# skywind3000/QuickNet

Hardware: AMD Instinct MI355X
Metric: RS(k,m) FEC encode+decode GiB/s (device-resident) at 1/2/4/8 MI355X (higher is better)
Workload: dtype u8

## Files before the change

### quicknet_amd/csrc/gf256.cpp

```cpp
#include <string.h>

#include <algorithm>
#include <mutex>
#include <vector>

#include "qfec_internal.hpp"

namespace qfec {

namespace {

uint8_t clmul_reduce(uint8_t a, uint8_t b) {
    unsigned acc = 0, x = a;
    for (int i = 0; i < 8; ++i)
        if (b & (1u << i)) acc ^= x << i;
    for (int bit = 14; bit >= 8; --bit)
        if (acc & (1u << bit)) acc ^= 0x11Du << (bit - 8);
    return (uint8_t)acc;
}

Field g_field;
std::once_flag g_field_once;

void build_field() {
    Field& f = g_field;
    for (int a = 0; a < 256; ++a)
        for (int b = 0; b < 256; ++b) f.mul[a][b] = clmul_reduce((uint8_t)a, (uint8_t)b);
    uint8_t x = 1;
    memset(f.log, 0, sizeof(f.log));
    for (int i = 0; i < 255; ++i) {
        f.exp[i] = x;
        f.exp[i + 255] = x;
        f.log[x] = (uint8_t)i;
        x = f.mul[x][2];
    }
    f.exp[510] = f.exp[511] = 0;
    f.log[0] = 255;
    f.inv[0] = 0;
    for (int a = 1; a < 256; ++a) f.inv[a] = f.exp[(255 - f.log[a]) % 255];
}

}

Tuning& tuning() {
    static Tuning t;
    return t;
}

const Field& field() {
    std::call_once(g_field_once, build_field);
    return g_field;
}

DivMagic make_div_magic(uint32_t d) {
    DivMagic m{};
    if (d == 0) d = 1;
    if ((d & (d - 1)) == 0) {
        m.pow2 = 1;
        m.shift = 0;
        while ((1u << m.shift) < d) ++m.shift;
        m.mul = 1;
        return m;
    }
    uint32_t l = 0;
    while ((1ull << l) < d) ++l;
    m.pow2 = 0;
    m.shift = l;
    m.mul = (uint64_t)(((unsigned __int128)1 << (32 + l)) / d) + 1;
    return m;
}

bool gf_invert(uint8_t* a, int k) {
    const Field& f = field();
    std::vector<uint8_t> aug((size_t)k * 2 * k, 0);
    const int w = 2 * k;
    for (int r = 0; r < k; ++r) {
        memcpy(&aug[(size_t)r * w], a + (size_t)r * k, (size_t)k);
        aug[(size_t)r * w + k + r] = 1;
    }
    for (int c = 0; c < k; ++c) {
        int p = c;
        while (p < k && aug[(size_t)p * w + c] == 0) ++p;
        if (p == k) return false;
        if (p != c)
            for (int j = 0; j < w; ++j) std::swap(aug[(size_t)p * w + j], aug[(size_t)c * w + j]);
        uint8_t* pr = &aug[(size_t)c * w];
        const uint8_t s = f.inv[pr[c]];
        for (int j = 0; j < w; ++j) pr[j] = f.mul[s][pr[j]];
        for (int r = 0; r < k; ++r) {
            if (r == c) continue;
            uint8_t* rr = &aug[(size_t)r * w];
            const uint8_t q = rr[c];
            if (!q) continue;
            const uint8_t* mq = f.mul[q];
            for (int j = 0; j < w; ++j) rr[j] ^= mq[pr[j]];
        }
    }
    for (int r = 0; r < k; ++r) memcpy(a + (size_t)r * k, &aug[(size_t)r * w + k], (size_t)k);
    return true;
}

bool gf_invert_rs(uint8_t* a, int k) {
    const Field& f = field();
    std::vector<uint8_t> used((size_t)k, 0);
    std::vector<int> sw_row((size_t)k, -1), sw_col((size_t)k, -1);
    auto row = [&](int r) { return a + (size_t)r * k; };
    for (int s = 0; s < k; ++s) {
        int pr = -1, pc = -1;
        if (!used[s] && row(s)[s]) {
            pr = pc = s;
        } else {
            for (int r = 0; r < k && pc < 0; ++r) {
                if (used[r]) continue;
                for (int c = 0; c < k; ++c)
                    if (!used[c] && row(r)[c]) { pr = r; pc = c; break; }
            }
            if (pc < 0) return false;
        }
        used[pc] = 1;
        if (pr != pc) std::swap_ranges(row(pr), row(pr) + k, row(pc));
        sw_row[s] = pr;
        sw_col[s] = pc;
        uint8_t* p = row(pc);
        if (p[pc] != 1) {
            const uint8_t* sc = f.mul[f.inv[p[pc]]];
            p[pc] = 1;
            for (int c = 0; c < k; ++c) p[c] = sc[p[c]];
        }
        bool unit = true;
        for (int c = 0; c < k && unit; ++c) unit = p[c] == (c == pc);
        if (unit) continue;
        for (int r = 0; r < k; ++r) {
            if (r == pc) continue;
            uint8_t* q = row(r);
            const uint8_t x = q[pc];
            q[pc] = 0;
            if (!x) continue;
            const uint8_t* mx = f.mul[x];
            for (int c = 0; c < k; ++c) q[c] ^= mx[p[c]];
        }
    }
    for (int s = k - 1; s >= 0; --s)
        if (sw_row[s] != sw_col[s])
            for (int r = 0; r < k; ++r) std::swap(row(r)[sw_row[s]], row(r)[sw_col[s]]);
    return true;
}

bool cauchy_rows(int k, int m, std::vector<uint8_t>& out) {
    if (k <= 0 || m <= 0 || k + m > 255) return false;
    const Field& f = field();
    out.assign((size_t)m * k, 0);
    for (int j = 0; j < m; ++j)
        for (int i = 0; i < k; ++i) out[(size_t)j * k + i] = f.inv[(m + i) ^ j];
    return true;
}

bool vandermonde_rows(int k, int m, std::vector<uint8_t>& out) {
    const int n = k + m;
    if (k <= 0 || m < 0 || k > 256 || n > 256) return false;
    const Field& f = field();
    std::vector<uint8_t> v((size_t)n * k, 0);
    v[0] = 1;
    for (int r = 1; r < n; ++r)
        for (int c = 0; c < k; ++c) v[(size_t)r * k + c] = f.exp[((r - 1) * c) % 255];
    std::vector<uint8_t> top(v.begin(), v.begin() + (size_t)k * k);
    if (!gf_invert(top.data(), k)) return false;
    out.assign((size_t)m * k, 0);
    for (int r = 0; r < m; ++r)
        for (int c = 0; c < k; ++c) {
            uint8_t acc = 0;
            const uint8_t* row = &v[(size_t)(k + r) * k];
            for (int i = 0; i < k; ++i) acc ^= f.mul[row[i]][top[(size_t)i * k + c]];
            out[(size_t)r * k + c] = acc;
        }
    return true;
}

static inline uint32_t pack4(uint8_t a, uint8_t b, uint8_t c, uint8_t d) {
    return (uint32_t)a | ((uint32_t)b << 8) | ((uint32_t)c << 16) | ((uint32_t)d << 24);
}

void perm_entry(uint8_t c, uint32_t* o) {
    const Field& f = field();
    const uint8_t* mc = f.mul[c];
    o[0] = pack4(mc[0], mc[1], mc[2], mc[3]);
    o[1] = pack4(mc[4], mc[5], mc[6], mc[7]);
    o[2] = pack4(mc[0], mc[8], mc[16], mc[24]);
    o[3] = pack4(mc[32], mc[40], mc[48], mc[56]);
    o[4] = pack4(mc[0], mc[64], mc[128], mc[192]);
    o[5] = 0;
    o[6] = c ? f.log[c] : 0xFFu;
    o[7] = c;
}

int decode_rows(const uint8_t* P, int k, int m, const uint8_t* marks, std::vector<uint8_t>& rows,
                std::vector<int>& survivors, std::vector<int>& lost, const uint8_t* full) {
    lost.clear();
    survivors.clear();
    for (int i = 0; i < k; ++i) {
        if (marks[i]) lost.push_back(i);
        else survivors.push_back(i);
    }
    const int e = (int)lost.size();
    if (e == 0) return 0;
    for (int j = 0; j < m && (int)survivors.size() < k; ++j)
        if (!marks[k + j]) survivors.push_back(k + j);
    if ((int)survivors.size() < k) return -1;
    std::vector<uint8_t> d((size_t)k * k, 0);
    if (full) {
        for (int r = 0; r < k; ++r) memcpy(&d[(size_t)r * k], full + (size_t)survivors[r] * k, (size_t)k);
        (void)gf_invert_rs(d.data(), k);
    } else {
        for (int r = 0; r < k; ++r) {
            const int s = survivors[r];
            if (s < k) d[(size_t)r * k + s] = 1;
            else memcpy(&d[(size_t)r * k], P + (size_t)(s - k) * k, (size_t)k);
        }
        if (!gf_invert(d.data(), k)) return -1;
    }
    rows.assign((size_t)e * k, 0);
    for (int j = 0; j < e; ++j) memcpy(&rows[(size_t)j * k], &d[(size_t)lost[j] * k], (size_t)k);
    return e;
}

int repair_rows(const uint8_t* P, int k, int m, const uint8_t* marks, std::vector<uint8_t>& rows,
                std::vector<int>& survivors, std::vector<int>& lost, const uint8_t* full, int* e_out) {
    const int n = k + m;
    int t = 0;
    for (int i = 0; i < n; ++i) t += marks[i] ? 1 : 0;
    rows.clear();
    survivors.clear();
    lost.clear();
    if (e_out) *e_out = 0;
    if (t == 0) return 0;
    if (t > m) return -1;
    std::vector<uint8_t> drows;
    std::vector<int> dlost;
    const int e = decode_rows(P, k, m, marks, drows, survivors, dlost, full);
    if (e < 0) return -1;
    if (e_out) *e_out = e;
    lost = dlost;
    for (int j = 0; j < m; ++j)
        if (marks[k + j]) lost.push_back(k + j);
    rows.assign((size_t)t * k, 0);
    if (e) memcpy(rows.data(), drows.data(), (size_t)e * k);
    const Field& f = field();
    std::vector<int> pos((size_t)k, -1);
    for (int c = 0; c < k; ++c)
        if (survivors[c] < k) pos[survivors[c]] = c;
    for (int r = e; r < t; ++r) {
        const uint8_t* pr = P + (size_t)(lost[r] - k) * k;
        uint8_t* out = &rows[(size_t)r * k];
        for (int i = 0; i < k; ++i)
            if (pos[i] >= 0) out[pos[i]] ^= pr[i];
        for (int j = 0; j < e; ++j) {
            const uint8_t q = pr[dlost[j]];
            if (!q) continue;
            const uint8_t* mq = f.mul[q];
            for (int c = 0; c < k; ++c) out[c] ^= mq[drows[(size_t)j * k + c]];
        }
    }
    return t;
}

void build_repair_record(const RecordLayout& L, int k, int t, int e, const uint8_t* rows, const int* survivors,
                         const int* lost, bool rs_quirk, uint32_t* out) {
    memset(out, 0, (size_t)L.hdr * sizeof(uint32_t));
    out[0] = (uint32_t)t;
    out[2] = (uint32_t)e;
    for (int c = 0; c < k; ++c) out[L.surv_off + c] = (uint32_t)survivors[c];
    for (int j = 0; j < t; ++j) out[L.lost_off + j] = (uint32_t)lost[j];
    for (int j = 0; j < t; ++j)
        for (int c = 0; c < k; ++c) out[L.coff + j * k + c] = (uint32_t)rows[(size_t)j * k + c] * (QFEC_TAB_STRIDE * 4);
    if (rs_quirk)
        for (int j = 0; j < e && j < 32; ++j)
            if (rows[(size_t)j * k] == 0) out[1] |= 1u << j;
}

RecordLayout record_layout(int k, int m) {
    RecordLayout L;
    L.surv_off = 4;
    L.lost_off = 4 + k;
    L.coff = (4 + k + m + 7) & ~7;
    L.hdr = (L.coff + m * k + 7) & ~7;
    return L;
}

void build_record(const RecordLayout& L, int k, int e, const uint8_t* rows, const int* survivors,
                  const int* lost, bool rs_quirk, uint32_t* out) {
    memset(out, 0, L.words(e, k) * sizeof(uint32_t));
    out[0] = (uint32_t)e;
    for (int c = 0; c < k; ++c) out[L.surv_off + c] = (uint32_t)survivors[c];
    for (int j = 0; j < e; ++j) out[L.lost_off + j] = (uint32_t)lost[j];
    for (int j = 0; j < e; ++j)
        for (int c = 0; c < k; ++c) {
            uint32_t* t = out + L.hdr + ((size_t)j * k + c) * QFEC_TAB_STRIDE;
            perm_entry(rows[(size_t)j * k + c], t);
            out[L.coff + j * k + c] = (uint32_t)rows[(size_t)j * k + c] * (QFEC_TAB_STRIDE * 4);
        }
    if (rs_quirk)
        for (int j = 0; j < e; ++j)
            if (rows[(size_t)j * k] == 0) {
                out[L.hdr + ((size_t)j * k) * QFEC_TAB_STRIDE + 5] = 1;
                if (j < 32) out[1] |= 1u << j;
            }
}

}
```

### quicknet_amd/csrc/qfec_internal.hpp

```cpp
#pragma once

#include <hip/hip_runtime.h>
#include <stdint.h>

#include <atomic>
#include <vector>

namespace qfec {

constexpr int QFEC_TAB_STRIDE = 8;

constexpr int QFEC_REC_NONE = -1;
constexpr int QFEC_REC_FAIL = -2;
constexpr int QFEC_LE_UNCHECKED = -1;
constexpr int QFEC_LE_LOST = -2;
constexpr int QFEC_LUT_MAX_N = 24;

constexpr int QFEC_VARIANT_PERM_I = 0;
constexpr int QFEC_VARIANT_LDSLOG_I = 1;

struct DivMagic {
    uint64_t mul;
    uint32_t shift;
    uint32_t pow2;
};

DivMagic make_div_magic(uint32_t d);

struct EncodeArgs {
    const uint8_t* data;
    uint8_t* parity;
    const uint32_t* tab;
    const uint8_t* gf_exp;
    const uint8_t* gf_log;
    uint64_t work;
    uint64_t pitch;
    uint64_t dgs, pgs;
    DivMagic cols_div;
    uint32_t cols;
    int k, m;
    int vec16;
    int impl;
    int lds;
    int block;
};

struct ReconArgs {
    uint8_t* data;
    const uint8_t* parity;
    const uint8_t* marks;
    const int32_t* lut;
    const int32_t* group_rec;
    const uint32_t* records;
    unsigned int* failed;
    uint64_t groups;
    uint64_t pitch;
    uint64_t dgs, pgs;
    uint32_t cols;
    int k, m;
    int surv_off, lost_off, hdr;
    int coff;
    const uint32_t* t256;
    int vec16;
    int impl;
    uint32_t wpg;
    uint32_t cols8, wpg8;
    uint32_t cols12, wpg12;
    int rlds;
};

struct RepairArgs {
    uint8_t* data;
    uint8_t* parity;
    const uint8_t* dmarks;
    const uint8_t* pmarks;
    const int32_t* lut;
    const uint32_t* records;
    const uint32_t* t256;
    unsigned int* failed;
    uint64_t groups;
    uint64_t pitch;
    uint64_t dgs, pgs;
    uint32_t cols;
    uint32_t cols8, wpg8;
    int k, m;
    int surv_off, lost_off, coff;
    int vec16;
};

struct VerifyArgs {
    const uint8_t* data;
    const uint8_t* parity;
    const uint32_t* tab;
    unsigned int* bad_rows;
    unsigned int* bad_groups;
    uint64_t work;
    uint64_t pitch;
    uint64_t dgs, pgs;
    DivMagic cols_div;
    uint32_t cols;
    uint32_t block;
    int k, m;
    int vec16;
};

struct LocateArgs {
    const uint8_t* data;
    const uint8_t* parity;
    const uint32_t* tab;
    const uint32_t* rtab;
    unsigned int* bad_rows;
    unsigned int* cand;
    uint64_t work;
    uint64_t pitch;
    uint64_t dgs, pgs;
    DivMagic cols_div;
    uint32_t cols;
    uint32_t block;
    int k, m;
    int vec16;
};

struct LocateFinishArgs {
    const unsigned int* bad_rows;
    const unsigned int* cand;
    int* culprit;
    uint8_t* marks;
    unsigned int* counts;
    uint64_t groups;
    int k, m;
};

struct LocErasedArgs {
    const uint8_t* data;
    const uint8_t* parity;
    const uint8_t* dmarks;
    const uint8_t* pmarks;
    const int32_t* lut;
    const uint32_t* records;
    const uint32_t* t256;
    unsigned int* bad;
    unsigned int* cand;
    uint64_t groups;
    uint64_t pitch;
    uint64_t dgs, pgs;
    uint32_t cols;
    uint32_t cols8, wpg8;
    uint32_t block;
    int k, m;
    int ids_off, aoff, roff;
    int vec16;
};

struct LocErasedFinishArgs {
    const uint8_t* marks;
    const int32_t* lut;
    const uint32_t* records;
    const unsigned int* bad;
    const unsigned int* cand;
    int* culprit;
    uint8_t* marks_out;
    unsigned int* counts;
    uint64_t groups;
    int k, m;
    int ids_off;
    int scrub;
};

struct WireArgs {
    const uint8_t* payload;
    const int64_t* offsets;
    const int32_t* sizes;
    const uint32_t* seq;
    uint8_t* shards;
    uint64_t group_stride;
    uint64_t pitch;
    uint8_t* wire;
    uint64_t wire_pitch;
    int32_t* wire_len;
    uint8_t* marks;
    int32_t* rx_size;
    int32_t* status;
    int32_t* psize;
    uint64_t groups;
    int k, m;
    int checksum;
    int dec_pkt_size;
    int store_nt;
};

hipError_t launch_build_shards(const WireArgs& a, hipStream_t s);
hipError_t launch_pack_fused(const WireArgs& a, const uint32_t* tab, uint32_t* part, hipStream_t s, bool* launched);
struct FrameArgs {
    const uint8_t* in;
    const int32_t* in_len;
    uint8_t* out;
    int32_t* out_len;
    const uint8_t* mask;
    uint32_t* conv_hid;
    int32_t* status;
    uint8_t* info;
    uint64_t rows, in_pitch, out_pitch;
    uint32_t gmask, cmd, protocol;
    int session;
};
hipError_t launch_frame_udp(const FrameArgs& a, hipStream_t s);
struct FrameSend {
    const uint8_t* mask;
    const uint32_t* conv_hid;
    uint32_t gmask, cmd, protocol;
};
struct FrameRecv {
    uint32_t gmask;
    int32_t* status;
    uint32_t* conv_hid;
};
hipError_t launch_pack_frames(const WireArgs& a, const FrameSend& fs, int fp, const uint32_t* tab, hipStream_t s,
                              bool* launched);
hipError_t launch_unpack_frames(const WireArgs& a, const FrameRecv& fr, int fp, const int32_t* lut,
                                const uint32_t* records, uint32_t rec_hdr, hipStream_t s, bool* launched);
hipError_t launch_len_by_status(int32_t* len, const int32_t* status, uint64_t rows, hipStream_t s);
hipError_t launch_gather_rows(const uint8_t* base, const uint64_t* off, const int32_t* len, uint64_t rows, int wrap_n,
                              int wrap_k, uint8_t* out, uint64_t out_pitch, int32_t* out_len, hipStream_t s);
hipError_t launch_rx(const WireArgs& a, const int32_t* lut, const uint32_t* records, uint32_t rec_hdr, hipStream_t s,
                     bool* launched);
hipError_t launch_unframe_udp(const FrameArgs& a, hipStream_t s);
hipError_t launch_emit_wire(const WireArgs& a, hipStream_t s);
hipError_t launch_parse_wire(const WireArgs& a, hipStream_t s);
hipError_t launch_check_payloads(const WireArgs& a, hipStream_t s);

struct Tuning {
    std::atomic<int> recon_impl{-1};
    std::atomic<int> encode_impl{-1};
    std::atomic<int> wire_fused{1};
    std::atomic<int> wire_rx{1};
    std::atomic<int> host_chunk{0};
    std::atomic<int> host_threads{0};
    std::atomic<int> host_zero_copy{1};
    std::atomic<int> host_lanes{4};
    std::atomic<int> host_nt{2};
    std::atomic<int> encode_block{-1};
    std::atomic<int> encode_lds{-1};
};
Tuning& tuning();

hipError_t launch_encode(const EncodeArgs& a, int variant, hipStream_t stream);
hipError_t launch_reconstruct(const ReconArgs& a, hipStream_t stream);
hipError_t launch_repair(const RepairArgs& a, hipStream_t stream);
hipError_t launch_verify(const VerifyArgs& a, hipStream_t stream);
hipError_t launch_locate(const LocateArgs& a, hipStream_t stream);
hipError_t launch_locate_finish(const LocateFinishArgs& a, hipStream_t stream);
hipError_t launch_locate_erased(const LocErasedArgs& a, hipStream_t stream);
hipError_t launch_locate_erased_finish(const LocErasedFinishArgs& a, hipStream_t stream);
hipError_t launch_synth_fill(uint8_t* p, uint64_t nbytes, uint64_t seed, hipStream_t stream);
hipError_t launch_probe_xor(const EncodeArgs& a, hipStream_t stream);
hipError_t launch_probe_recon(const ReconArgs& a, hipStream_t stream);

struct Field {
    uint8_t exp[512];
    uint8_t log[256];
    uint8_t inv[256];
    uint8_t mul[256][256];
};

const Field& field();

bool cauchy_rows(int k, int m, std::vector<uint8_t>& out);
bool vandermonde_rows(int k, int m, std::vector<uint8_t>& out);

bool gf_invert(uint8_t* a, int k);
bool gf_invert_rs(uint8_t* a, int k);

void perm_entry(uint8_t c, uint32_t* out8);

int decode_rows(const uint8_t* parity_rows, int k, int m, const uint8_t* marks_n,
                std::vector<uint8_t>& rows, std::vector<int>& survivors, std::vector<int>& lost,
                const uint8_t* full = nullptr);

struct RecordLayout {
    int surv_off, lost_off, coff, hdr;
    size_t words(int e, int k) const { return (size_t)hdr + (size_t)e * k * QFEC_TAB_STRIDE; }
};
RecordLayout record_layout(int k, int m);

int repair_rows(const uint8_t* parity_rows, int k, int m, const uint8_t* marks_n, std::vector<uint8_t>& rows,
                std::vector<int>& survivors, std::vector<int>& lost, const uint8_t* full = nullptr,
                int* e_out = nullptr);
void build_repair_record(const RecordLayout& L, int k, int t, int e, const uint8_t* rows, const int* survivors,
                         const int* lost, bool rs_quirk, uint32_t* out);
void build_record(const RecordLayout& L, int k, int e, const uint8_t* rows, const int* survivors,
                  const int* lost, bool rs_quirk, uint32_t* out);

struct LocErasedLayout {
    int ids_off, aoff, roff, words;
};
LocErasedLayout loc_erased_layout(int k, int m);

}
```

### quicknet_amd/csrc/qfec_kernels.hip

```cpp
#include <hip/hip_runtime.h>
#include <stdint.h>

#include <algorithm>

#include "qfec_internal.hpp"

namespace qfec {

}
#include "qfec_device.hpp"
namespace qfec {


template <int K, int M, int BS = 256>
__global__ void __launch_bounds__(256) k_encode_perm(EncodeArgs a) {
    const uint64_t t = (uint64_t)blockIdx.x * (uint64_t)BS + threadIdx.x;
    if (t >= a.work) return;
    const uint64_t g = fast_div(t, a.cols_div);
    const uint32_t col = (uint32_t)(t - g * (uint64_t)a.cols);
    const uint8_t* src = a.data + g * a.dgs + (uint64_t)col * 16u;
    uint8_t* dst = a.parity + g * a.pgs + (uint64_t)col * 16u;
    const uint32_t* __restrict__ tab = a.tab;

    uint4 x[K];
#pragma unroll
    for (int c = 0; c < K; ++c) x[c] = ld16(src + (uint64_t)c * a.pitch);

    uint4 acc[M];
#pragma unroll
    for (int r = 0; r < M; ++r) {
        acc[r] = make_uint4(0, 0, 0, 0);
        if (tab[(r * K) * QFEC_TAB_STRIDE + 5]) acc[r] = *reinterpret_cast<const uint4*>(dst + (uint64_t)r * a.pitch);
    }
#pragma unroll
    for (int c = 0; c + 1 < K; c += 2) {
        Sel sa[4], sb[4];
        sel16(sa, x[c]);
        sel16(sb, x[c + 1]);
#pragma unroll
        for (int r = 0; r < M; ++r)
            gf_mac16x2(acc[r], sa, sb, tab + (r * K + c) * QFEC_TAB_STRIDE, tab + (r * K + c + 1) * QFEC_TAB_STRIDE);
    }
    if (K & 1) {
        Sel s[4];
        sel16(s, x[K - 1]);
#pragma unroll
        for (int r = 0; r < M; ++r) gf_mac16(acc[r], s, tab + (r * K + K - 1) * QFEC_TAB_STRIDE);
    }
#pragma unroll
    for (int r = 0; r < M; ++r) st16(dst + (uint64_t)r * a.pitch, acc[r]);
}

template <int K, int M, int BS = 256>
__global__ void __launch_bounds__(256) k_encode_perm_halves(EncodeArgs a) {
    constexpr int H = (K + 1) / 2;
    const uint64_t t = (uint64_t)blockIdx.x * (uint64_t)BS + threadIdx.x;
    if (t >= a.work) return;
    const uint64_t g = fast_div(t, a.cols_div);
    const uint32_t col = (uint32_t)(t - g * (uint64_t)a.cols);
    const uint8_t* src = a.data + g * a.dgs + (uint64_t)col * 16u;
    uint8_t* dst = a.parity + g * a.pgs + (uint64_t)col * 16u;
    const uint32_t* __restrict__ tab = a.tab;
    uint4 acc[M];
#pragma unroll
    for (int r = 0; r < M; ++r) {
        acc[r] = make_uint4(0, 0, 0, 0);
        if (tab[(r * K) * QFEC_TAB_STRIDE + 5]) acc[r] = *reinterpret_cast<const uint4*>(dst + (uint64_t)r * a.pitch);
    }
#pragma unroll
    for (int c0 = 0; c0 < K; c0 += H) {
        __builtin_amdgcn_sched_barrier(0);
        constexpr int HH = H;
        const int n = min(HH, K - c0);
        uint4 x[H];
#pragma unroll
        for (int i = 0; i < H; ++i)
            if (i < n) x[i] = ld16(src + (uint64_t)(c0 + i) * a.pitch);
#pragma unroll
        for (int i = 0; i + 1 < H; i += 2) {
            if (i + 1 >= n) continue;
            Sel sa[4], sb[4];
            sel16(sa, x[i]);
            sel16(sb, x[i + 1]);
#pragma unroll
            for (int r = 0; r < M; ++r)
                gf_mac16x2(acc[r], sa, sb, tab + (r * K + c0 + i) * QFEC_TAB_STRIDE,
                           tab + (r * K + c0 + i + 1) * QFEC_TAB_STRIDE);
        }
        if (n & 1) {
            Sel sl[4];
            sel16(sl, x[n - 1]);
#pragma unroll
            for (int r = 0; r < M; ++r) gf_mac16(acc[r], sl, tab + (r * K + c0 + n - 1) * QFEC_TAB_STRIDE);
        }
    }
#pragma unroll
    for (int r = 0; r < M; ++r) st16(dst + (uint64_t)r * a.pitch, acc[r]);
}

constexpr int RCH = 4;

__global__ void __launch_bounds__(256) k_encode_perm_any(EncodeArgs a) {
    const uint64_t t = (uint64_t)blockIdx.x * 256u + threadIdx.x;
    if (t >= a.work) return;
    const uint64_t g = fast_div(t, a.cols_div);
    const uint32_t col = (uint32_t)(t - g * (uint64_t)a.cols);
    const int k = a.k, m = a.m;
    const uint8_t* src = a.data + g * a.dgs + (uint64_t)col * 16u;
    uint8_t* dst = a.parity + g * a.pgs + (uint64_t)col * 16u;
    for (int r0 = 0; r0 < m; r0 += RCH) {
        uint4 acc[RCH];
#pragma unroll
        for (int j = 0; j < RCH; ++j) {
            acc[j] = make_uint4(0, 0, 0, 0);
            if (r0 + j < m && a.tab[((r0 + j) * k) * QFEC_TAB_STRIDE + 5])
                acc[j] = *reinterpret_cast<const uint4*>(dst + (uint64_t)(r0 + j) * a.pitch);
        }
        for (int c = 0; c < k; ++c) {
            const uint4 v = ld16(src + (uint64_t)c * a.pitch);
            Sel s[4];
            sel16(s, v);
#pragma unroll
            for (int j = 0; j < RCH; ++j)
                if (r0 + j < m) gf_mac16(acc[j], s, a.tab + ((r0 + j) * k + c) * QFEC_TAB_STRIDE);
        }
#pragma unroll
        for (int j = 0; j < RCH; ++j)
            if (r0 + j < m) st16(dst + (uint64_t)(r0 + j) * a.pitch, acc[j]);
    }
}

__global__ void __launch_bounds__(256) k_encode_bytes(EncodeArgs a) {
    const uint64_t t = (uint64_t)blockIdx.x * 256u + threadIdx.x;
    if (t >= a.work) return;
    const uint64_t g = fast_div(t, a.cols_div);
    const uint32_t b = (uint32_t)(t - g * (uint64_t)a.cols);
    const int k = a.k, m = a.m;
    const uint8_t* src = a.data + g * a.dgs + b;
    uint8_t* dst = a.parity + g * a.pgs + b;
    for (int r = 0; r < m; ++r) {
        const uint32_t* tr = a.tab + (r * k) * QFEC_TAB_STRIDE;
        uint32_t acc = tr[5] ? (uint32_t)dst[(uint64_t)r * a.pitch] : 0u;
        for (int c = 0; c < k; ++c) {
            const uint32_t* tc = tr + c * QFEC_TAB_STRIDE;
            const Sel s = gf_sel((uint32_t)src[(uint64_t)c * a.pitch]);
            acc ^= gf_mul4(s, tc[0], tc[1], tc[2], tc[3], tc[4]);
        }
        dst[(uint64_t)r * a.pitch] = (uint8_t)acc;
    }
}


__global__ void __launch_bounds__(256) k_encode_ldslog(EncodeArgs a) {
    __shared__ uint8_t s_exp[512];
    __shared__ uint8_t s_log[256];
    for (int i = threadIdx.x; i < 512; i += 256) s_exp[i] = a.gf_exp[i];
    s_log[threadIdx.x] = a.gf_log[threadIdx.x];
    __syncthreads();
    const uint64_t t = (uint64_t)blockIdx.x * 256u + threadIdx.x;
    if (t >= a.work) return;
    const uint64_t g = fast_div(t, a.cols_div);
    const uint32_t col = (uint32_t)(t - g * (uint64_t)a.cols);
    const int k = a.k, m = a.m;
    const uint8_t* src = a.data + g * a.dgs + (uint64_t)col * 16u;
    uint8_t* dst = a.parity + g * a.pgs + (uint64_t)col * 16u;
    for (int r0 = 0; r0 < m; r0 += RCH) {
        uint32_t acc[RCH][4];
#pragma unroll
        for (int j = 0; j < RCH; ++j) {
            uint4 init = make_uint4(0, 0, 0, 0);
            if (r0 + j < m && a.tab[((r0 + j) * k) * QFEC_TAB_STRIDE + 5])
                init = *reinterpret_cast<const uint4*>(dst + (uint64_t)(r0 + j) * a.pitch);
            acc[j][0] = init.x; acc[j][1] = init.y; acc[j][2] = init.z; acc[j][3] = init.w;
        }
        for (int c = 0; c < k; ++c) {
            const uint4 v = ld16(src + (uint64_t)c * a.pitch);
            const uint32_t w[4] = {v.x, v.y, v.z, v.w};
#pragma unroll
            for (int q = 0; q < 4; ++q) {
#pragma unroll
                for (int byte = 0; byte < 4; ++byte) {
                    const uint32_t x = (w[q] >> (8 * byte)) & 0xFFu;
                    const uint32_t lx = s_log[x];
#pragma unroll
                    for (int j = 0; j < RCH; ++j) {
                        if (r0 + j >= m) continue;
                        const uint32_t lc = a.tab[((r0 + j) * k + c) * QFEC_TAB_STRIDE + 6];
                        if (lc == 0xFFu) continue;
                        const uint32_t p = x ? (uint32_t)s_exp[lx + lc] : 0u;
                        acc[j][q] ^= p << (8 * byte);
                    }
                }
            }
        }
#pragma unroll
        for (int j = 0; j < RCH; ++j)
            if (r0 + j < m) st16(dst + (uint64_t)(r0 + j) * a.pitch, make_uint4(acc[j][0], acc[j][1], acc[j][2], acc[j][3]));
    }
}


__device__ __forceinline__ const uint8_t* shard_ptr(const ReconArgs& a, uint64_t g, uint32_t s) {
    return s < (uint32_t)a.k ? a.data + g * a.dgs + (uint64_t)s * a.pitch
                             : a.parity + g * a.pgs + (uint64_t)(s - a.k) * a.pitch;
}

__device__ __forceinline__ int group_record(const ReconArgs& a, uint64_t g, int lane) {
    int rec;
    if (a.group_rec) {
        rec = a.group_rec[g];
    } else {
        const int n = a.k + a.m;
        uint32_t mk = 0;
        if (lane < a.k) mk = a.marks[g * (uint64_t)a.k + lane];
        else if (lane < n) mk = a.marks[(uint64_t)a.groups * a.k + g * (uint64_t)a.m + (lane - a.k)];
        const uint64_t bal = __ballot(mk != 0);
        const uint32_t mask = (uint32_t)(bal & ((1ull << n) - 1ull));
        rec = a.lut[mask];
    }
    return __builtin_amdgcn_readfirstlane(rec);
}

template <int D>
__device__ __forceinline__ void stv(uint8_t* p, const uint32_t (&v)[D]) {
    if constexpr (D == 4) {
        const u32x4 t = {v[0], v[1], v[2], v[3]};
        __builtin_nontemporal_store(t, reinterpret_cast<u32x4*>(p));
    } else if constexpr (D == 3) {
        uint32_t* q = reinterpret_cast<uint32_t*>(p);
        __builtin_nontemporal_store(v[0], q);
        __builtin_nontemporal_store(v[1], q + 1);
        __builtin_nontemporal_store(v[2], q + 2);
    } else {
        const u32x2 t = {v[0], v[1]};
        __builtin_nontemporal_store(t, reinterpret_cast<u32x2*>(p));
    }
}
template <int D>
__device__ __forceinline__ void ldv_plain(uint32_t (&v)[D], const uint8_t* p) {
#pragma unroll
    for (int d = 0; d < D; ++d) v[d] = reinterpret_cast<const uint32_t*>(p)[d];
}

template <int K, int E, int D>
__device__ __forceinline__ void recon_column_e(const uint8_t* const (&src)[K], uint8_t* __restrict__ data_g,
                                               uint64_t lost_bits, const RTab& T, uint64_t pitch, uint64_t off) {
    uint32_t x[K][D];
#pragma unroll
    for (int c = 0; c < K; ++c) ldv<D>(x[c], src[c] + off);
    uint8_t* dst[E];
    uint32_t acc[E][D];
#pragma unroll
    for (int j = 0; j < E; ++j) {
        const uint32_t l = (uint32_t)__builtin_ctzll(lost_bits);
        lost_bits &= lost_bits - 1;
        dst[j] = data_g + (uint64_t)l * pitch + off;
#pragma unroll
        for (int d = 0; d < D; ++d) acc[j][d] = 0;
        if (T.quirk(j, K)) ldv_plain<D>(acc[j], dst[j]);
    }
    recon_mac_core<K, E, D>(x, acc, T);
#pragma unroll
    for (int j = 0; j < E; ++j) stv<D>(dst[j], acc[j]);
}

template <int K, int M, int D, int E = M>
__device__ __forceinline__ void recon_column_by_e(const uint8_t* const (&src)[K], uint8_t* __restrict__ data_g,
                                                  uint64_t lost_bits, const RTab& T, int e, uint64_t pitch, uint64_t off) {
    if constexpr (E > 1) {
        if (e < E) {
            recon_column_by_e<K, M, D, E - 1>(src, data_g, lost_bits, T, e, pitch, off);
            return;
        }
    }
    recon_column_e<K, E, D>(src, data_g, lost_bits, T, pitch, off);
}

template <int K, int M, int IMPL>
__device__ __forceinline__ void recon_item(const ReconArgs& a, uint8_t* __restrict__ data,
                                           const uint8_t* __restrict__ parity, const uint8_t* __restrict__ marks,
                                           const int32_t* __restrict__ lut, const uint32_t* __restrict__ records,
                                           uint32_t wid, int lane) {
    constexpr int N = K + M;
    const uint32_t wpg = IMPL == 3 ? a.wpg8 : IMPL == 4 ? a.wpg12 : a.wpg;
    const uint64_t g = wid / wpg;
    const uint32_t part = wid - (uint32_t)g * wpg;
    if (g >= a.groups) return;
    uint32_t mk = 0;
    if (lane < K) mk = marks[g * K + lane];
    else if (lane < N) mk = marks[a.groups * K + g * M + (lane - K)];
    const uint64_t mask = __ballot(mk != 0) & ((1ull << N) - 1ull);
    const uint64_t lost_bits = mask & ((1ull << K) - 1ull);
    const int e = __builtin_popcountll(lost_bits);
    if (e == 0) return;
    uint64_t avail = ~mask & ((1ull << N) - 1ull);
    if (__builtin_popcountll(avail) < K) {
        if (part == 0 && lane == 0 && a.failed) atomicAdd(a.failed, 1u);
        return;
    }
    const int rec = ((const __attribute__((address_space(4))) int32_t*)lut)[mask];
    const RTab T{records + rec, a.coff, a.t256};
    const uint64_t pitch = a.pitch;
    uint8_t* data_g = data + g * a.dgs;
    const uint8_t* par_g = parity + g * a.pgs;
    const uint8_t* src[K];
#pragma unroll
    for (int c = 0; c < K; ++c) {
        const uint32_t s = (uint32_t)__builtin_ctzll(avail);
        avail &= avail - 1;
        src[c] = s < (uint32_t)K ? data_g + (uint64_t)s * pitch : par_g + (uint64_t)(s - K) * pitch;
    }
    const uint32_t col = part * 64u + lane;
    if (col < (IMPL == 3 ? a.cols8 : IMPL == 4 ? a.cols12 : a.cols)) {
        if (IMPL == 2) recon_column_by_e<K, M, 4>(src, data_g, lost_bits, T, e, pitch, (uint64_t)col * 16u);
        else if (IMPL == 3) recon_column_by_e<K, M, 2>(src, data_g, lost_bits, T, e, pitch, (uint64_t)col * 8u);
        else recon_column_by_e<K, M, 3>(src, data_g, lost_bits, T, e, pitch, (uint64_t)col * 12u);
    }
}

template <int K, int M, int IMPL_>
__global__ void __launch_bounds__(256) k_reconstruct_perm(ReconArgs a, uint8_t* __restrict__ data,
                                                          const uint8_t* __restrict__ parity,
                                                          const uint8_t* __restrict__ marks,
                                                          const int32_t* __restrict__ lut,
                                                          const uint32_t* __restrict__ records) {
    constexpr int IMPL = IMPL_ == 8 ? 3 : IMPL_;
    const int lane = threadIdx.x & 63;
    const uint32_t wid = __builtin_amdgcn_readfirstlane(blockIdx.x * (IMPL_ == 8 ? a.wpg8 : 4u) + (threadIdx.x >> 6));
    recon_item<K, M, IMPL>(a, data, parity, marks, lut, records, wid, lane);
}

template <bool VEC16>
__global__ void __launch_bounds__(256) k_reconstruct_any(ReconArgs a) {
    const int lane = threadIdx.x & 63;
    const uint64_t g = (uint64_t)blockIdx.x * 4u + (threadIdx.x >> 6);
    if (g >= a.groups) return;
    const int rec = group_record(a, g, lane);
    if (rec < 0) {
        if (rec == QFEC_REC_FAIL && lane == 0 && a.failed) atomicAdd(a.failed, 1u);
        return;
    }
    const uint32_t* __restrict__ r = a.records + rec;
    const int e = (int)r[0];
    const int k = a.k;
    const uint32_t* surv = r + a.surv_off;
    const uint32_t* lost = r + a.lost_off;
    const uint32_t* tab = r + a.hdr;

    for (uint32_t col = lane; col < (uint32_t)a.cols; col += 64) {
        for (int j0 = 0; j0 < e; j0 += RCH) {
            if (VEC16) {
                const uint64_t off = (uint64_t)col * 16u;
                uint4 acc[RCH];
#pragma unroll
                for (int j = 0; j < RCH; ++j) {
                    acc[j] = make_uint4(0, 0, 0, 0);
                    const int jj = j0 + j;
                    if (jj < e && tab[(jj * k) * QFEC_TAB_STRIDE + 5])
                        acc[j] = *reinterpret_cast<const uint4*>(a.data + g * a.dgs + (uint64_t)lost[jj] * a.pitch + off);
                }
                for (int c = 0; c < k; ++c) {
                    const uint4 v = ld16(shard_ptr(a, g, surv[c]) + off);
                    Sel s[4];
                    sel16(s, v);
#pragma unroll
                    for (int j = 0; j < RCH; ++j)
                        if (j0 + j < e) gf_mac16(acc[j], s, tab + ((j0 + j) * k + c) * QFEC_TAB_STRIDE);
                }
#pragma unroll
                for (int j = 0; j < RCH; ++j)
                    if (j0 + j < e) st16(a.data + g * a.dgs + (uint64_t)lost[j0 + j] * a.pitch + off, acc[j]);
            } else {
                const uint64_t off = col;
                uint32_t acc[RCH];
#pragma unroll
                for (int j = 0; j < RCH; ++j) {
                    acc[j] = 0;
                    const int jj = j0 + j;
                    if (jj < e && tab[(jj * k) * QFEC_TAB_STRIDE + 5])
                        acc[j] = a.data[g * a.dgs + (uint64_t)lost[jj] * a.pitch + off];
                }
                for (int c = 0; c < k; ++c) {
                    const Sel s = gf_sel((uint32_t)shard_ptr(a, g, surv[c])[off]);
#pragma unroll
                    for (int j = 0; j < RCH; ++j)
                        if (j0 + j < e) {
                            const uint32_t* tc = tab + ((j0 + j) * k + c) * QFEC_TAB_STRIDE;
                            acc[j] ^= gf_mul4(s, tc[0], tc[1], tc[2], tc[3], tc[4]);
                        }
                }
#pragma unroll
                for (int j = 0; j < RCH; ++j)
                    if (j0 + j < e) a.data[g * a.dgs + (uint64_t)lost[j0 + j] * a.pitch + off] = (uint8_t)acc[j];
            }
        }
    }
}


template <int K, int T, int D>
__device__ __forceinline__ void repair_column_t(const uint8_t* const (&src)[K], uint8_t* __restrict__ data_g,
                                                uint8_t* __restrict__ par_g, uint64_t lost_bits, const RTab& R,
                                                uint64_t pitch, uint64_t off) {
    uint32_t x[K][D];
#pragma unroll
    for (int c = 0; c < K; ++c) ldv<D>(x[c], src[c] + off);
    uint8_t* dst[T];
    uint32_t acc[T][D];
#pragma unroll
    for (int j = 0; j < T; ++j) {
        const uint32_t l = (uint32_t)__builtin_ctzll(lost_bits);
        lost_bits &= lost_bits - 1;
        dst[j] = (l < (uint32_t)K ? data_g + (uint64_t)l * pitch : par_g + (uint64_t)(l - K) * pitch) + off;
#pragma unroll
        for (int d = 0; d < D; ++d) acc[j][d] = 0;
        if (R.quirk(j, K)) ldv_plain<D>(acc[j], dst[j]);
    }
    recon_mac_core<K, T, D>(x, acc, R);
#pragma unroll
    for (int j = 0; j < T; ++j) stv<D>(dst[j], acc[j]);
}

template <int K, int M, int D, int T = M>
__device__ __forceinline__ void repair_column_by_t(const uint8_t* const (&src)[K], uint8_t* __restrict__ data_g,
                                                   uint8_t* __restrict__ par_g, uint64_t lost_bits, const RTab& R,
                                                   int t, uint64_t pitch, uint64_t off) {
    if constexpr (T > 1) {
        if (t < T) {
            repair_column_by_t<K, M, D, T - 1>(src, data_g, par_g, lost_bits, R, t, pitch, off);
            return;
        }
    }
    repair_column_t<K, T, D>(src, data_g, par_g, lost_bits, R, pitch, off);
}

template <int K, int M, bool ONE>
__global__ void __launch_bounds__(256) k_repair_perm(RepairArgs a, uint8_t* __restrict__ data,
                                                     uint8_t* __restrict__ parity,
                                                     const uint8_t* __restrict__ dmarks,
                                                     const uint8_t* __restrict__ pmarks,
                                                     const int32_t* __restrict__ lut,
                                                     const uint32_t* __restrict__ records) {
    constexpr int N = K + M;
    const int lane = threadIdx.x & 63;
    const uint32_t wave = __builtin_amdgcn_readfirstlane(threadIdx.x >> 6);
    uint64_t g;
    uint32_t part;
    if (ONE) {
        g = blockIdx.x;
        part = wave;
    } else {
        const uint32_t wid = blockIdx.x * 4u + wave;
        g = wid / a.wpg8;
        part = wid - (uint32_t)g * a.wpg8;
    }
    if (g >= a.groups) return;
    uint32_t mk = 0;
    if (lane < K) mk = dmarks[g * K + lane];
    else if (lane < N) mk = pmarks[g * M + (lane - K)];
    const uint64_t mask = __ballot(mk != 0) & ((1ull << N) - 1ull);
    const int t = __builtin_popcountll(mask);
    if (t == 0) return;
    if (t > M) {
        if (part == 0 && lane == 0 && a.failed) atomicAdd(a.failed, 1u);
        return;
    }
    const int rec = ((const __attribute__((address_space(4))) int32_t*)lut)[mask];
    if (rec < 0) {
        if (part == 0 && lane == 0 && a.failed) atomicAdd(a.failed, 1u);
        return;
    }
    const RTab R{records + rec, a.coff, a.t256};
    const uint64_t pitch = a.pitch;
    uint8_t* data_g = data + g * a.dgs;
    uint8_t* par_g = parity + g * a.pgs;
    uint64_t avail = ~mask & ((1ull << N) - 1ull);
    const uint8_t* src[K];
#pragma unroll
    for (int c = 0; c < K; ++c) {
        const uint32_t s = (uint32_t)__builtin_ctzll(avail);
        avail &= avail - 1;
        src[c] = s < (uint32_t)K ? data_g + (uint64_t)s * pitch : par_g + (uint64_t)(s - K) * pitch;
    }
    const uint32_t col = part * 64u + lane;
    if (col < a.cols8) repair_column_by_t<K, M, 2>(src, data_g, par_g, mask, R, t, pitch, (uint64_t)col * 8u);
}

template <bool VEC16>
__global__ void __launch_bounds__(256) k_repair_any(RepairArgs a) {
    const int lane = threadIdx.x & 63;
    const uint64_t g = (uint64_t)blockIdx.x * 4u + (threadIdx.x >> 6);
    if (g >= a.groups) return;
    const int k = a.k, m = a.m, n = k + m;
    uint32_t mk = 0;
    if (lane < k) mk = a.dmarks[g * (uint64_t)k + lane];
    else if (lane < n) mk = a.pmarks[g * (uint64_t)m + (lane - k)];
    const uint32_t mask = (uint32_t)(__ballot(mk != 0) & ((1ull << n) - 1ull));
    if (!mask) return;
    const int rec = __builtin_amdgcn_readfirstlane(a.lut[mask]);
    if (rec < 0) {
        if (rec == QFEC_REC_FAIL && lane == 0 && a.failed) atomicAdd(a.failed, 1u);
        return;
    }
    const uint32_t* __restrict__ r = a.records + rec;
    const int t = (int)r[0];
    const uint32_t quirk = r[1];
    const uint32_t* surv = r + a.surv_off;
    const uint32_t* lost = r + a.lost_off;
    const uint32_t* offs = r + a.coff;
    uint8_t* data_g = a.data + g * a.dgs;
    uint8_t* par_g = a.parity + g * a.pgs;
    auto row = [&](uint32_t s) -> uint8_t* {
        return s < (uint32_t)k ? data_g + (uint64_t)s * a.pitch : par_g + (uint64_t)(s - k) * a.pitch;
    };

    for (uint32_t col = lane; col < a.cols; col += 64) {
        for (int j0 = 0; j0 < t; j0 += RCH) {
            if (VEC16) {
                const uint64_t off = (uint64_t)col * 16u;
                uint4 acc[RCH];
#pragma unroll
                for (int j = 0; j < RCH; ++j) {
                    acc[j] = make_uint4(0, 0, 0, 0);
                    const int jj = j0 + j;
                    if (jj < t && ((quirk >> jj) & 1u)) acc[j] = *reinterpret_cast<const uint4*>(row(lost[jj]) + off);
                }
                for (int c = 0; c < k; ++c) {
                    const uint4 v = ld16(row(surv[c]) + off);
                    Sel s[4];
                    sel16(s, v);
#pragma unroll
                    for (int j = 0; j < RCH; ++j)
                        if (j0 + j < t) gf_mac16(acc[j], s, a.t256 + (offs[(j0 + j) * k + c] >> 2));
                }
#pragma unroll
                for (int j = 0; j < RCH; ++j)
                    if (j0 + j < t) st16(row(lost[j0 + j]) + off, acc[j]);
            } else {
                const uint64_t off = col;
                uint32_t acc[RCH];
#pragma unroll
                for (int j = 0; j < RCH; ++j) {
                    acc[j] = 0;
                    const int jj = j0 + j;
                    if (jj < t && ((quirk >> jj) & 1u)) acc[j] = row(lost[jj])[off];
                }
                for (int c = 0; c < k; ++c) {
                    const Sel s = gf_sel((uint32_t)row(surv[c])[off]);
#pragma unroll
                    for (int j = 0; j < RCH; ++j)
                        if (j0 + j < t) {
                            const uint32_t* tc = a.t256 + (offs[(j0 + j) * k + c] >> 2);
                            acc[j] ^= gf_mul4(s, tc[0], tc[1], tc[2], tc[3], tc[4]);
                        }
                }
#pragma unroll
                for (int j = 0; j < RCH; ++j)
                    if (j0 + j < t) row(lost[j0 + j])[off] = (uint8_t)acc[j];
            }
        }
    }
}


__global__ void __launch_bounds__(256) k_synth_fill(uint8_t* p, uint64_t nbytes, uint64_t seed) {
    const uint64_t j = (uint64_t)blockIdx.x * 256u + threadIdx.x;
    const uint64_t nwords = (nbytes + 7) / 8;
    if (j >= nwords) return;
    uint64_t z = seed + (j + 1) * 0x9E3779B97F4A7C15ull;
    z = (z ^ (z >> 30)) * 0xBF58476D1CE4E5B9ull;
    z = (z ^ (z >> 27)) * 0x94D049BB133111EBull;
    z = z ^ (z >> 31);
    const uint64_t base = j * 8;
    if (base + 8 <= nbytes && ((reinterpret_cast<uintptr_t>(p) & 7u) == 0)) {
        *reinterpret_cast<uint64_t*>(p + base) = z;
    } else {
        for (int i = 0; i < 8 && base + i < nbytes; ++i) p[base + i] = (uint8_t)(z >> (8 * i));
    }
}

template <int BS = 256>
__global__ void __launch_bounds__(256) k_probe_xor(EncodeArgs a) {
    const uint64_t t = (uint64_t)blockIdx.x * (uint64_t)BS + threadIdx.x;
    if (t >= a.work) return;
    const uint64_t g = fast_div(t, a.cols_div);
    const uint32_t col = (uint32_t)(t - g * (uint64_t)a.cols);
    const uint8_t* src = a.data + g * a.dgs + (uint64_t)col * 16u;
    uint8_t* dst = a.parity + g * a.pgs + (uint64_t)col * 16u;
    uint4 acc = make_uint4(0, 0, 0, 0);
    for (int c0 = 0; c0 < a.k; c0 += 16) {
        uint4 v[16];
#pragma unroll
        for (int c = 0; c < 16; ++c)
            if (c0 + c < a.k) v[c] = ld16(src + (uint64_t)(c0 + c) * a.pitch);
#pragma unroll
        for (int c = 0; c < 16; ++c)
            if (c0 + c < a.k) { acc.x ^= v[c].x; acc.y ^= v[c].y; acc.z ^= v[c].z; acc.w ^= v[c].w; }
    }
    for (int r = 0; r < a.m; ++r) {
        st16(dst + (uint64_t)r * a.pitch, acc);
        acc.x += 1u;
    }
}

template <int K, int M>
__global__ void __launch_bounds__(256) k_probe_recon(ReconArgs a) {
    constexpr int N = K + M;
    const int lane = threadIdx.x & 63;
    const uint64_t g = blockIdx.x;
    const uint32_t part = __builtin_amdgcn_readfirstlane(threadIdx.x >> 6);
    uint32_t mk = 0;
    if (lane < K) mk = a.marks[g * K + lane];
    else if (lane < N) mk = a.marks[a.groups * K + g * M + (lane - K)];
    const uint64_t mask = __ballot(mk != 0) & ((1ull << N) - 1ull);
    uint64_t lost = mask & ((1ull << K) - 1ull);
    if (!lost) return;
    uint64_t avail = ~mask & ((1ull << N) - 1ull);
    if (__builtin_popcountll(avail) < K) return;
    const uint32_t col = part * 64u + lane;
    if (col >= a.cols8) return;
    const uint64_t off = (uint64_t)col * 8u;
    uint8_t* data_g = a.data + g * a.dgs;
    const uint8_t* par_g = a.parity + g * a.pgs;
    uint32_t x[K][2];
#pragma unroll
    for (int c = 0; c < K; ++c) {
        const uint32_t s = (uint32_t)__builtin_ctzll(avail);
        avail &= avail - 1;
        ldv<2>(x[c], (s < (uint32_t)K ? data_g + (uint64_t)s * a.pitch : par_g + (uint64_t)(s - K) * a.pitch) + off);
    }
    uint32_t acc[2] = {0, 0};
#pragma unroll
    for (int c = 0; c < K; ++c) { acc[0] ^= x[c][0]; acc[1] ^= x[c][1]; }
    while (lost) {
        const uint32_t l = (uint32_t)__builtin_ctzll(lost);
        lost &= lost - 1;
        stv<2>(data_g + (uint64_t)l * a.pitch + off, acc);
        acc[0] += 1u;
    }
}

hipError_t launch_probe_recon(const ReconArgs& a, hipStream_t stream) {
    if (a.groups == 0) return hipSuccess;
    if (a.wpg8 < 1 || a.wpg8 > 4 || a.groups > 0x7FFFFFFFull) return hipErrorInvalidValue;
#define QFEC_PROBE_REC(KK, MM)                                                                                    \
    if (a.k == KK && a.m == MM) {                                                                                 \
        hipLaunchKernelGGL((k_probe_recon<KK, MM>), dim3((unsigned)a.groups), dim3(64 * a.wpg8),               \
                           (size_t)std::max(a.rlds, 0), stream, a);                                               \
        return hipGetLastError();                                                                                 \
    }
    QFEC_PROBE_REC(10, 3)
    QFEC_PROBE_REC(16, 4)
#undef QFEC_PROBE_REC
    return hipErrorInvalidValue;
}


static inline unsigned grid_for(uint64_t work, unsigned block) {
    return (unsigned)((work + block - 1) / block);
}

static inline unsigned enc_block(const EncodeArgs& a, int K, int im) {
    if (a.block == 64 || a.block == 256) return (unsigned)a.block;
    const bool lines = (a.pitch % 128 == 0) && (a.dgs % 128 == 0) && (a.pgs % 128 == 0) &&
                       ((reinterpret_cast<uintptr_t>(a.data) | reinterpret_cast<uintptr_t>(a.parity)) % 128 == 0);
    return im == 0 && K >= 6 && K <= 10 && a.m <= 3 && a.cols >= 64 && lines && a.work >= (8192ull << 8) ? 64u : 256u;
}

static inline size_t enc_lds(const EncodeArgs& a, int K, int im, unsigned grid, unsigned bs = 256) {
    if (a.lds >= 0) return (size_t)a.lds;
    if (bs == 64) return 16384;
    if (grid < 8192 || K <= 2) return 0;
    if (im == 0 && K == 10) return a.cols >= 32 && grid >= 16384 ? 65536 : 40960;
    if (im == 2 && a.cols <= 64) return 27000;
    return 40960;
}

#define QFEC_ENC_CASE(KK, MM)                                                                 \
    if (a.k == KK && a.m == MM) {                                                             \
        const int im = a.impl < 0 ? (KK >= 16 ? 2 : 0) : a.impl;                              \
        const unsigned bs = enc_block(a, KK, im);                                             \
        const size_t lds = enc_lds(a, KK, im, grid, bs);                                      \
        if (im == 2 && bs == 64)                                                              \
            hipLaunchKernelGGL((k_encode_perm_halves<KK, MM, 64>), dim3(grid_for(a.work, 64)), dim3(64), lds, stream, a); \
        else if (im == 2)                                                                     \
            hipLaunchKernelGGL((k_encode_perm_halves<KK, MM>), dim3(grid), dim3(256), lds, stream, a); \
        else if (bs == 64)                                                                    \
            hipLaunchKernelGGL((k_encode_perm<KK, MM, 64>), dim3(grid_for(a.work, 64)), dim3(64), lds, stream, a); \
        else                                                                                  \
            hipLaunchKernelGGL((k_encode_perm<KK, MM>), dim3(grid), dim3(256), lds, stream, a);  \
        return hipGetLastError();                                                             \
    }

hipError_t launch_encode(const EncodeArgs& a, int variant, hipStream_t stream) {
    if (a.work == 0) return hipSuccess;
    const unsigned grid = grid_for(a.work, 256);
    if (!a.vec16) {
        hipLaunchKernelGGL(k_encode_bytes, dim3(grid), dim3(256), 0, stream, a);
        return hipGetLastError();
    }
    if (variant == QFEC_VARIANT_LDSLOG_I) {
        hipLaunchKernelGGL(k_encode_ldslog, dim3(grid), dim3(256), 0, stream, a);
        return hipGetLastError();
    }
    QFEC_ENC_CASE(10, 3)
    QFEC_ENC_CASE(16, 4)
    QFEC_ENC_CASE(4, 2)
    QFEC_ENC_CASE(2, 1)
    QFEC_ENC_CASE(2, 2)
    QFEC_ENC_CASE(3, 1)
    QFEC_ENC_CASE(3, 2)
    QFEC_ENC_CASE(4, 1)
    QFEC_ENC_CASE(5, 1)
    QFEC_ENC_CASE(5, 3)
    QFEC_ENC_CASE(6, 2)
    QFEC_ENC_CASE(7, 1)
    QFEC_ENC_CASE(8, 2)
    QFEC_ENC_CASE(8, 4)
    QFEC_ENC_CASE(12, 4)
    QFEC_ENC_CASE(20, 4)
    hipLaunchKernelGGL(k_encode_perm_any, dim3(grid), dim3(256), 0, stream, a);
    return hipGetLastError();
}

#define QFEC_REC_LAUNCH(KK, MM, AR)                                                                        \
    do {                                                                                                   \
        const dim3 blk(AR == 8 ? 64u * a.wpg8 : 256u), grd(AR == 8 ? (unsigned)a.groups : pgrid);          \
        hipLaunchKernelGGL((k_reconstruct_perm<KK, MM, AR>), grd, blk, 0, stream, a, a.data, a.parity, a.marks, \
                           a.lut, a.records);                                                              \
    } while (0)

#define QFEC_REC_CASE(KK, MM)                                                      \
    if (a.k == KK && a.m == MM) {                                                  \
         \
         \
         \
        const bool wide8 = KK >= 10 && fill8 >= fill16 - 0.01;                     \
        int im = a.impl < 0 ? (KK * MM <= 30 && lanes12 ? 4 : (lanes8 || wide8) ? 3 : 2) : a.impl; \
        if (im == 4 && !lanes12_ok) im = 2;                                        \
        const unsigned pgrid = im == 3 ? pgrid8 : im == 4 ? pgrid12 : pgrid16;     \
         \
         \
        if (im == 3 && a.impl < 0) im = 8;                                         \
        if (im == 8 && (a.wpg8 < 1 || a.wpg8 > 4)) im = 3;                         \
        if (im == 8) QFEC_REC_LAUNCH(KK, MM, 8);                                   \
        else if (im == 4) QFEC_REC_LAUNCH(KK, MM, 4);                              \
        else if (im == 3) QFEC_REC_LAUNCH(KK, MM, 3);                              \
        else QFEC_REC_LAUNCH(KK, MM, 2);                                           \
        return hipGetLastError();                                                  \
    }

hipError_t launch_reconstruct(const ReconArgs& a, hipStream_t stream) {
    if (a.groups == 0) return hipSuccess;
    const unsigned grid = grid_for(a.groups, 4);
    if (!a.vec16) {
        hipLaunchKernelGGL((k_reconstruct_any<false>), dim3(grid), dim3(256), 0, stream, a);
        return hipGetLastError();
    }
    if (a.group_rec) {
        hipLaunchKernelGGL((k_reconstruct_any<true>), dim3(grid), dim3(256), 0, stream, a);
        return hipGetLastError();
    }
    const uint64_t waves = a.groups * (uint64_t)std::max(std::max(a.wpg, a.wpg8), a.wpg12);
    if (waves > 0xFFFFFFFFull) return hipErrorInvalidValue;
    const unsigned pgrid16 = grid_for(a.groups * (uint64_t)a.wpg, 4);
    const unsigned pgrid8 = grid_for(a.groups * (uint64_t)a.wpg8, 4);
    const unsigned pgrid12 = grid_for(a.groups * (uint64_t)a.wpg12, 4);
    const bool lanes12_ok = a.cols12 * 12u <= a.cols * 16u;
    const double fill16 = (double)a.cols / (64.0 * a.wpg), fill8 = (double)a.cols8 / (64.0 * a.wpg8),
                 fill12 = (double)a.cols12 / (64.0 * a.wpg12);
    const bool lanes12 = lanes12_ok && fill12 > fill16 + 0.1 && fill12 >= fill8 - 0.01;
    const bool lanes8 = fill8 > fill16 + 0.1;
    QFEC_REC_CASE(10, 3)
    QFEC_REC_CASE(16, 4)
    QFEC_REC_CASE(4, 2)
    QFEC_REC_CASE(2, 1)
    QFEC_REC_CASE(3, 2)
    QFEC_REC_CASE(8, 4)
    QFEC_REC_CASE(12, 4)
    QFEC_REC_CASE(5, 3)
    QFEC_REC_CASE(6, 2)
    QFEC_REC_CASE(7, 1)
    QFEC_REC_CASE(8, 2)
    QFEC_REC_CASE(20, 4)
    hipLaunchKernelGGL((k_reconstruct_any<true>), dim3(grid), dim3(256), 0, stream, a);
    return hipGetLastError();
}

#define QFEC_REP_CASE(KK, MM)                                                                                   \
    if (a.k == KK && a.m == MM) {                                                                               \
        if (a.wpg8 >= 1 && a.wpg8 <= 4)                                                                         \
            hipLaunchKernelGGL((k_repair_perm<KK, MM, true>), dim3((unsigned)a.groups), dim3(64u * a.wpg8), 0, \
                               stream, a, a.data, a.parity, a.dmarks, a.pmarks, a.lut, a.records);              \
        else                                                                                                    \
            hipLaunchKernelGGL((k_repair_perm<KK, MM, false>), dim3(grid_for(a.groups * (uint64_t)a.wpg8, 4)), \
                               dim3(256), 0, stream, a, a.data, a.parity, a.dmarks, a.pmarks, a.lut, a.records); \
        return hipGetLastError();                                                                               \
    }

hipError_t launch_repair(const RepairArgs& a, hipStream_t stream) {
    if (a.groups == 0) return hipSuccess;
    if (a.k + a.m > QFEC_LUT_MAX_N) return hipErrorInvalidValue;
    if (a.groups * (uint64_t)std::max(a.wpg8, 1u) > 0x7FFFFFFFull) return hipErrorInvalidValue;
    const unsigned grid = grid_for(a.groups, 4);
    if (!a.vec16) {
        hipLaunchKernelGGL((k_repair_any<false>), dim3(grid), dim3(256), 0, stream, a);
        return hipGetLastError();
    }
    QFEC_REP_CASE(10, 3)
    QFEC_REP_CASE(16, 4)
    QFEC_REP_CASE(4, 2)
    QFEC_REP_CASE(2, 1)
    QFEC_REP_CASE(3, 2)
    QFEC_REP_CASE(8, 4)
    QFEC_REP_CASE(12, 4)
    QFEC_REP_CASE(5, 3)
    QFEC_REP_CASE(6, 2)
    QFEC_REP_CASE(7, 1)
    QFEC_REP_CASE(8, 2)
    QFEC_REP_CASE(20, 4)
    hipLaunchKernelGGL((k_repair_any<true>), dim3(grid), dim3(256), 0, stream, a);
    return hipGetLastError();
}

hipError_t launch_synth_fill(uint8_t* p, uint64_t nbytes, uint64_t seed, hipStream_t stream) {
    const uint64_t nwords = (nbytes + 7) / 8;
    if (!nwords) return hipSuccess;
    hipLaunchKernelGGL(k_synth_fill, dim3(grid_for(nwords, 256)), dim3(256), 0, stream, p, nbytes, seed);
    return hipGetLastError();
}

hipError_t launch_probe_xor(const EncodeArgs& a, hipStream_t stream) {
    if (a.work == 0) return hipSuccess;
    const unsigned grid = grid_for(a.work, 256);
    const unsigned bs = enc_block(a, a.k, 0);
    const size_t lds = bs == 64 && a.lds < 0 ? 27000 : enc_lds(a, a.k, 0, grid, bs);
    if (bs == 64)
        hipLaunchKernelGGL(k_probe_xor<64>, dim3(grid_for(a.work, 64)), dim3(64), lds, stream, a);
    else
        hipLaunchKernelGGL(k_probe_xor<>, dim3(grid), dim3(256), lds, stream, a);
    return hipGetLastError();
}

}
```

### quicknet_amd/csrc/qfec_repair.cpp

```cpp
#include "qfec_rt.hpp"

namespace qfec {

static int ensure_repair_lut(qfec_code* c, int dev, DevTables** out) {
    DevTables& d = c->dev[dev];
    *out = &d;
    if (d.rep_version == c->version && d.d_rep_lut) return QFEC_OK;
    const int k = c->k, m = c->m, n = k + m;
    const size_t nmask = (size_t)1 << n;
    const RecordLayout L = record_layout(k, m);
    std::vector<int32_t> lut(nmask);
    std::vector<uint32_t> recs;
    std::vector<uint8_t> marks((size_t)n), rows;
    std::vector<int> surv, lost;
    for (size_t mask = 0; mask < nmask; ++mask) {
        const int t = __builtin_popcountll((unsigned long long)mask);
        if (t == 0) { lut[mask] = QFEC_REC_NONE; continue; }
        if (t > m) { lut[mask] = QFEC_REC_FAIL; continue; }
        for (int i = 0; i < n; ++i) marks[i] = (mask >> i) & 1;
        int e = 0;
        if (repair_rows(c->rows.data(), k, m, marks.data(), rows, surv, lost, full_of(c), &e) != t) {
            lut[mask] = QFEC_REC_FAIL;
            continue;
        }
        const size_t off = recs.size();
        recs.resize(off + (size_t)L.hdr);
        build_repair_record(L, k, t, e, rows.data(), surv.data(), lost.data(), c->quirk != 0, &recs[off]);
        lut[mask] = (int32_t)off;
    }
    if (d.d_rep_lut) HIP_TRY(hipFree(d.d_rep_lut));
    if (d.d_rep_rec) HIP_TRY(hipFree(d.d_rep_rec));
    d.d_rep_lut = nullptr;
    d.d_rep_rec = nullptr;
    HIP_TRY(hipMalloc(&d.d_rep_lut, nmask * 4));
    HIP_TRY(hipMalloc(&d.d_rep_rec, std::max<size_t>(recs.size(), 8) * 4));
    HIP_TRY(hipMemcpy(d.d_rep_lut, lut.data(), nmask * 4, hipMemcpyHostToDevice));
    if (!recs.empty()) HIP_TRY(hipMemcpy(d.d_rep_rec, recs.data(), recs.size() * 4, hipMemcpyHostToDevice));
    d.rep_version = c->version;
    return QFEC_OK;
}

static int repair_unsupported(const qfec_code* c) {
    set_error("qfec_repair: k + m = %d > %d is not supported (no host-record path for repair)", c->k + c->m,
              QFEC_LUT_MAX_N);
    return QFEC_EUNSUP;
}

static int run_repair(DevCtx& ctx, const qfec_code* c, const DevTables& d, uint8_t* d_data, uint8_t* d_par,
                      const uint8_t* d_marks, long long groups, int block, long long pitch, unsigned* d_failed,
                      hipStream_t s) {
    RepairArgs a{};
    const RecordLayout L = record_layout(c->k, c->m);
    a.lut = d.d_rep_lut;
    a.records = d.d_rep_rec;
    a.t256 = ctx.d_t256;
    a.failed = d_failed;
    a.pitch = (uint64_t)pitch;
    a.k = c->k;
    a.m = c->m;
    a.surv_off = L.surv_off;
    a.lost_off = L.lost_off;
    a.coff = L.coff;
    a.dgs = (uint64_t)c->k * pitch;
    a.pgs = (uint64_t)c->m * pitch;
    a.vec16 = vec16_ok(d_data, d_par, block, pitch) ? 1 : 0;
    a.cols = a.vec16 ? (uint32_t)((block + 15) / 16) : (uint32_t)block;
    a.cols8 = a.vec16 && c->k < 14 ? 2u * a.cols : (uint32_t)((block + 7) / 8);
    a.wpg8 = (a.cols8 + 63) / 64;
    const long long per = std::max<long long>(1, 0x7FFFFFFFll / (long long)std::max(a.wpg8, 1u));
    for (long long g0 = 0; g0 < groups; g0 += per) {
        const long long gn = std::min(per, groups - g0);
        a.data = d_data + (size_t)g0 * a.dgs;
        a.parity = d_par + (size_t)g0 * a.pgs;
        a.dmarks = d_marks + (size_t)g0 * c->k;
        a.pmarks = d_marks + (size_t)groups * c->k + (size_t)g0 * c->m;
        a.groups = (uint64_t)gn;
        hipError_t e = launch_repair(a, s);
        if (e != hipSuccess) return hip_fail(e, "repair kernel launch");
    }
    return QFEC_OK;
}

}

using namespace qfec;

extern "C" {

int qfec_prepare_repair(qfec_code* code) {
    if (!code) return QFEC_EINVAL;
    if (code->k + code->m > QFEC_LUT_MAX_N) return repair_unsupported(code);
    DevCtx* ctx = nullptr;
    int rc = current_ctx(&ctx);
    if (rc) return rc;
    DevTables* d = nullptr;
    std::lock_guard<std::mutex> lk(code->mu);
    return ensure_repair_lut(code, ctx->device, &d);
}

int qfec_repair(qfec_code* code, unsigned char* d_data, unsigned char* d_parity, const unsigned char* d_marks,
                long long groups, int block_size, long long pitch, unsigned int* d_failed, void* stream) {
    if (!code || groups < 0 || block_size < 1 || pitch < block_size ||
        (groups > 0 && (!d_data || !d_marks || (code->m > 0 && !d_parity)))) {
        set_error("qfec_repair: invalid argument");
        return QFEC_EINVAL;
    }
    if (code->k + code->m > QFEC_LUT_MAX_N) return repair_unsupported(code);
    if (groups == 0) return QFEC_OK;
    DevCtx* ctx = nullptr;
    int rc = current_ctx(&ctx);
    if (rc) return rc;
    DevTables* d = nullptr;
    {
        std::lock_guard<std::mutex> lk(code->mu);
        rc = ensure_repair_lut(code, ctx->device, &d);
    }
    if (rc) return rc;
    return run_repair(*ctx, code, *d, d_data, d_parity, d_marks, groups, block_size, pitch, d_failed,
                      (hipStream_t)stream);
}

int qfec_repair_rows(const qfec_code* code, const unsigned char* marks_n, unsigned char* rows_out,
                     int* survivors_out, int* lost_out) {
    if (!code || !marks_n) return QFEC_EINVAL;
    std::vector<uint8_t> rows;
    std::vector<int> surv, lost;
    const int t = repair_rows(code->rows.data(), code->k, code->m, marks_n, rows, surv, lost, full_of(code));
    if (t > 0) {
        if (rows_out) memcpy(rows_out, rows.data(), rows.size());
        if (survivors_out) memcpy(survivors_out, surv.data(), surv.size() * sizeof(int));
        if (lost_out) memcpy(lost_out, lost.data(), lost.size() * sizeof(int));
    }
    return t;
}

int qfec_verify(qfec_code* code, const unsigned char* d_data, const unsigned char* d_parity, long long groups,
                int block_size, long long pitch, unsigned int* d_bad_rows, unsigned int* d_bad_groups,
                void* stream) {
    if (!code || groups < 0 || block_size < 1 || pitch < block_size ||
        (groups > 0 && (!d_data || (code->m > 0 && !d_parity)))) {
        set_error("qfec_verify: invalid argument");
        return QFEC_EINVAL;
    }
    if (code->m > 32) {
        set_error("qfec_verify: m = %d > 32 (one bit per parity row in a 32-bit word)", code->m);
        return QFEC_EUNSUP;
    }
    if (groups == 0 || (!d_bad_rows && !d_bad_groups)) return QFEC_OK;
    DevCtx* ctx = nullptr;
    int rc = current_ctx(&ctx);
    if (rc) return rc;
    hipStream_t s = (hipStream_t)stream;
    unsigned* rows = d_bad_rows;
    if (!rows && hipMallocAsync((void**)&rows, (size_t)groups * 4, s) != hipSuccess)
        return hip_fail(hipGetLastError(), "verify scratch");
    auto done = [&](int r) {
        if (!d_bad_rows) (void)hipFreeAsync(rows, s);
        return r;
    };
    hipError_t he = hipMemsetAsync(rows, 0, (size_t)groups * 4, s);
    if (he != hipSuccess) return done(hip_fail(he, "verify: zeroing bad_rows"));
    if (code->m == 0) return done(QFEC_OK);
    uint32_t* tab = nullptr;
    {
        std::lock_guard<std::mutex> lk(code->mu);
        rc = ensure_enc(code, ctx->device, &tab);
    }
    if (rc) return done(rc);
    VerifyArgs a{};
    a.tab = tab;
    a.bad_groups = d_bad_groups;
    a.k = code->k;
    a.m = code->m;
    a.pitch = (uint64_t)pitch;
    a.block = (uint32_t)block_size;
    a.dgs = (uint64_t)code->k * pitch;
    a.pgs = (uint64_t)code->m * pitch;
    a.vec16 = vec16_ok(d_data, d_parity, block_size, pitch) ? 1 : 0;
    a.cols = a.vec16 ? (uint32_t)((block_size + 15) / 16) : (uint32_t)block_size;
    a.cols_div = make_div_magic(a.cols);
    const long long per = std::max<long long>(1, (long long)(0x7FFFFFFFll / a.cols));
    for (long long g0 = 0; g0 < groups; g0 += per) {
        const long long gn = std::min(per, groups - g0);
        a.data = d_data + (size_t)g0 * a.dgs;
        a.parity = d_parity + (size_t)g0 * a.pgs;
        a.bad_rows = rows + g0;
        a.work = (uint64_t)gn * a.cols;
        he = launch_verify(a, s);
        if (he != hipSuccess) return done(hip_fail(he, "verify kernel launch"));
    }
    return done(QFEC_OK);
}

}
```

### quicknet_amd/csrc/qfec_rt.hpp

```cpp
#pragma once

#include <hip/hip_runtime.h>
#include <stdarg.h>
#include <stdio.h>
#include <stdlib.h>
#include <string.h>

#include <algorithm>
#include <atomic>
#include <chrono>
#include <functional>
#include <map>
#include <memory>
#include <mutex>
#include <string>
#include <unordered_map>
#include <unordered_set>
#include <vector>

#include "../../include/qfec.h"
#include "../../include/qfec_fec.h"
#include "../../include/qfec_rs.h"
#include "qfec_internal.hpp"
#include "qfec_maps.hpp"
#include "qfec_percall.hpp"
#include "qfec_pool.hpp"

namespace qfec {

extern thread_local std::string t_last_error;
void set_error(const char* fmt, ...) __attribute__((format(printf, 1, 2)));
int hip_fail(hipError_t e, const char* what);

#define HIP_TRY(expr)                                       \
    do {                                                    \
        hipError_t _e = (expr);                             \
        if (_e != hipSuccess) return hip_fail(_e, #expr);   \
    } while (0)

inline size_t round_up(size_t x, size_t a) { return (x + a - 1) / a * a; }

extern std::atomic<int> g_variant;
extern std::atomic<int> g_percall_fast, g_percall_resident, g_percall_idle_us, g_percall_timeout_us,
    g_percall_fault, g_percall_group, g_percall_stop_us;
extern std::atomic<unsigned long long> g_group_hits, g_group_misses;

constexpr int kMaxDevices = 64;
constexpr int kMaxHostLanes = 8;

struct DevCtx {
    int device = 0;
    std::mutex mu;
    hipStream_t stream = nullptr;
    uint8_t* d_stage = nullptr;
    size_t d_cap = 0;
    uint8_t* h_stage = nullptr;
    size_t h_cap = 0;
    uint8_t* d_gf = nullptr;
    uint32_t* d_t256 = nullptr;
    uint32_t* d_small = nullptr;
    size_t small_cap = 0;
    uint32_t* h_small = nullptr;
    unsigned* d_counter = nullptr;
    uint8_t* h_pc = nullptr;
    uint8_t* d_pc = nullptr;
    size_t pc_cap = 0;
    uint32_t* h_pc_done = nullptr;
    uint32_t* d_pc_done = nullptr;
    uint32_t pc_seq = 0;
    uint32_t pc_unsynced = 0;
    struct PcServer {
        int usable = 0;
        hipStream_t stream = nullptr;
        PcBell* bell = nullptr;
        uint8_t* in = nullptr;
        uint8_t* h_out = nullptr;
        uint8_t* d_out = nullptr;
        PcStatus* h_st = nullptr;
        PcStatus* d_st = nullptr;
        uint32_t req = 0;
        uint32_t tab_last[kPcTabWords];
        size_t tab_bytes = 0;
        uint32_t gen = 0;
        bool launched = false;
        unsigned long long calls = 0, launches = 0, relaunches = 0, timeouts = 0, abandoned = 0;
        unsigned long long tr[7] = {0, 0, 0, 0, 0, 0, 0};
    } srv;
    int init_rc = QFEC_ENODEV;
    struct HostSlot {
        hipStream_t stream = nullptr;
        hipEvent_t done = nullptr;
        uint8_t* d_buf = nullptr;
        uint8_t* h_in = nullptr;
        uint8_t* h_out = nullptr;
        size_t in_cap = 0, out_cap = 0;
    } host[kMaxHostLanes];
    std::mutex host_mu;
};

extern DevCtx g_ctx[kMaxDevices];

int current_ctx(DevCtx** out);
int ensure_stage(DevCtx& c, size_t dbytes, size_t hbytes);
int ensure_pc(DevCtx& c, size_t bytes);
int ensure_small(DevCtx& c, size_t words);
bool is_device_ptr(const void* p);
bool is_pinned_host(const void* p);
bool host_dev(const void* h, uint8_t** d);
int ensure_host_slot(DevCtx::HostSlot& h, size_t in_bytes, size_t out_bytes);
void quiesce_host_slots(DevCtx& c);
int gather_rows(DevCtx& c, unsigned char* const* ptrs, size_t count, int len, size_t pitch, uint8_t* d_dst,
                uint8_t* h_tmp, bool dev_src);
int scatter_rows(DevCtx& c, unsigned char* const* ptrs, size_t count, int len, size_t pitch, const uint8_t* d_src,
                 uint8_t* h_tmp, bool dev_dst, const uint8_t* only);

bool pc_server_alive(const DevCtx::PcServer& s);
hipError_t pc_server_stop(DevCtx& c, long long limit_us = -1);

}

struct DevTables {
    uint32_t* d_enc = nullptr;
    uint64_t enc_version = ~0ull;
    int32_t* d_lut = nullptr;
    uint32_t* d_rec = nullptr;
    uint64_t rec_version = ~0ull;
    int32_t* d_rep_lut = nullptr;
    uint32_t* d_rep_rec = nullptr;
    uint64_t rep_version = ~0ull;
    uint32_t* d_loc = nullptr;
    uint64_t loc_version = ~0ull;
    int32_t* d_le_lut = nullptr;
    uint32_t* d_le_rec = nullptr;
    uint64_t le_version = ~0ull;
};

struct qfec_code {
    int k = 0, m = 0;
    int quirk = 0;
    std::mutex mu;
    std::vector<uint8_t> rows;
    std::vector<uint8_t> full;
    uint64_t version = 0;
    std::map<int, DevTables> dev;
    std::unordered_map<uint64_t, std::vector<uint32_t>> rec_cache;
    uint64_t rec_cache_version = ~0ull;
    std::shared_ptr<const std::vector<uint8_t>> lut_seed;
    uint64_t lut_seed_version = ~0ull;
    uint64_t le_host_version = ~0ull;
    int le_rc = 0;
    std::string le_error;
    std::vector<uint32_t> le_recs;
    std::vector<std::pair<uint32_t, int32_t>> le_masks;
};

namespace qfec {

qfec_code* make_code(int k, int m, std::vector<uint8_t>&& rows, int quirk);
void free_code(qfec_code* c);
const uint8_t* full_of(const qfec_code* c);
int ensure_enc(qfec_code* c, int dev, uint32_t** out);
int ensure_lut(qfec_code* c, int dev, DevTables** out);
bool vec16_ok(const void* a, const void* b, int block, long long pitch);
int run_encode(DevCtx& ctx, const qfec_code* c, const uint32_t* tab, int m, const uint8_t* d_data, uint8_t* d_par,
               long long groups, int block, long long pitch, hipStream_t s, long long dgs = -1, long long pgs = -1,
               bool host_mem = false);
int run_reconstruct(DevCtx& ctx, const qfec_code* c, const int32_t* lut, const int32_t* group_rec,
                    const uint32_t* recs, uint8_t* d_data, const uint8_t* d_par, const uint8_t* d_marks,
                    long long groups, int block, long long pitch, unsigned* d_failed, hipStream_t s,
                    long long dgs = -1, long long pgs = -1);
int host_records(qfec_code* c, const uint8_t* marks, long long groups, std::vector<int32_t>& grec,
                 std::vector<uint32_t>& recs, long long* nfail);
int reconstruct_host_records(DevCtx& ctx, qfec_code* c, uint8_t* d_data, const uint8_t* d_par,
                             const uint8_t* d_marks, long long groups, int block_size, long long pitch,
                             unsigned* d_failed, hipStream_t s);

}
```

### quicknet_amd/csrc/qfec_runtime.cpp

```cpp
#include "qfec_rt.hpp"

#define QFEC_VERSION_STRING "qfec 0.1.0 (gfx950)"

using namespace qfec;

namespace qfec {

std::shared_ptr<HostPool> host_pool() {
    static std::mutex mu;
    static std::shared_ptr<HostPool> pool;
    static int made_with = -1;
    std::lock_guard<std::mutex> lk(mu);
    const int want = tuning().host_threads;
    if (!pool || want != made_with) {
        const int n = want > 0 ? std::min(want, 64) : std::min(usable_cpus(), 32);
        pool = std::make_shared<HostPool>(n);
        made_with = want;
    }
    return pool;
}

}

namespace qfec {

thread_local std::string t_last_error;

void set_error(const char* fmt, ...) {
    char buf[512];
    va_list ap;
    va_start(ap, fmt);
    vsnprintf(buf, sizeof(buf), fmt, ap);
    va_end(ap);
    t_last_error = buf;
}

int hip_fail(hipError_t e, const char* what) {
    set_error("%s: %s", what, hipGetErrorString(e));
    return QFEC_EHIP;
}

std::atomic<int> g_variant{QFEC_VARIANT_PERM};
std::atomic<int> g_percall_fast{1};
std::atomic<unsigned long long> g_group_hits{0}, g_group_misses{0};

DevCtx g_ctx[kMaxDevices];
std::once_flag g_ctx_once[kMaxDevices];

int init_ctx(DevCtx& c, int dev) {
    c.device = dev;
    HIP_TRY(hipSetDevice(dev));
    HIP_TRY(hipStreamCreateWithFlags(&c.stream, hipStreamNonBlocking));
    const Field& f = field();
    HIP_TRY(hipMalloc(&c.d_gf, 768));
    HIP_TRY(hipMemcpy(c.d_gf, f.exp, 512, hipMemcpyHostToDevice));
    HIP_TRY(hipMemcpy(c.d_gf + 512, f.log, 256, hipMemcpyHostToDevice));
    HIP_TRY(hipMalloc(&c.d_counter, 256));
    std::vector<uint32_t> t256(256 * QFEC_TAB_STRIDE);
    for (int v = 0; v < 256; ++v) perm_entry((uint8_t)v, &t256[(size_t)v * QFEC_TAB_STRIDE]);
    HIP_TRY(hipMalloc(&c.d_t256, t256.size() * 4));
    HIP_TRY(hipMemcpy(c.d_t256, t256.data(), t256.size() * 4, hipMemcpyHostToDevice));
    return QFEC_OK;
}

int current_ctx(DevCtx** out) {
    int ndev = 0;
    hipError_t e = hipGetDeviceCount(&ndev);
    if (e != hipSuccess || ndev <= 0) {
        set_error("no HIP device available (%s)", e == hipSuccess ? "0 devices" : hipGetErrorString(e));
        return QFEC_ENODEV;
    }
    int dev = 0;
    HIP_TRY(hipGetDevice(&dev));
    if (dev < 0 || dev >= kMaxDevices) {
        set_error("device %d out of range", dev);
        return QFEC_ENODEV;
    }
    DevCtx& c = g_ctx[dev];
    std::call_once(g_ctx_once[dev], [&] {
        int prev = 0;
        (void)hipGetDevice(&prev);
        c.init_rc = init_ctx(c, dev);
        (void)hipSetDevice(prev);
    });
    if (c.init_rc != QFEC_OK) {
        if (t_last_error.empty()) set_error("device %d context initialisation failed", dev);
        return c.init_rc;
    }
    *out = &c;
    return QFEC_OK;
}

int ensure_stage(DevCtx& c, size_t dbytes, size_t hbytes) {
    if (dbytes > c.d_cap) {
        if (c.d_stage) HIP_TRY(hipFree(c.d_stage));
        c.d_stage = nullptr;
        c.d_cap = 0;
        const size_t cap = round_up(std::max(dbytes, (size_t)1 << 20), 1 << 20);
        HIP_TRY(hipMalloc(&c.d_stage, cap));
        c.d_cap = cap;
    }
    if (hbytes > c.h_cap) {
        if (c.h_stage) HIP_TRY(hipHostFree(c.h_stage));
        c.h_stage = nullptr;
        c.h_cap = 0;
        const size_t cap = round_up(std::max(hbytes, (size_t)1 << 20), 1 << 20);
        HIP_TRY(hipHostMalloc(&c.h_stage, cap, hipHostMallocDefault));
        c.h_cap = cap;
    }
    return QFEC_OK;
}

int ensure_pc(DevCtx& c, size_t bytes) {
    if (!c.h_pc_done) {
        HIP_TRY(hipHostMalloc((void**)&c.h_pc_done, 256, hipHostMallocMapped | hipHostMallocCoherent));
        HIP_TRY(hipHostGetDevicePointer((void**)&c.d_pc_done, c.h_pc_done, 0));
        __atomic_store_n(c.h_pc_done, 0u, __ATOMIC_RELEASE);
    }
    if (bytes <= c.pc_cap) return QFEC_OK;
    if (c.h_pc) HIP_TRY(hipStreamSynchronize(c.stream));
    if (c.h_pc) HIP_TRY(hipHostFree(c.h_pc));
    c.h_pc = c.d_pc = nullptr;
    c.pc_cap = 0;
    const size_t cap = round_up(std::max(bytes, (size_t)1 << 16), 1 << 16);
    HIP_TRY(hipHostMalloc(&c.h_pc, cap, hipHostMallocMapped));
    HIP_TRY(hipHostGetDevicePointer((void**)&c.d_pc, c.h_pc, 0));
    c.pc_cap = cap;
    return QFEC_OK;
}

int ensure_small(DevCtx& c, size_t words) {
    if (words <= c.small_cap) return QFEC_OK;
    if (c.d_small) HIP_TRY(hipFree(c.d_small));
    if (c.h_small) HIP_TRY(hipHostFree(c.h_small));
    c.d_small = nullptr;
    c.h_small = nullptr;
    c.small_cap = 0;
    const size_t cap = round_up(words, 4096);
    HIP_TRY(hipMalloc(&c.d_small, cap * 4));
    HIP_TRY(hipHostMalloc(&c.h_small, cap * 4, hipHostMallocDefault));
    c.small_cap = cap;
    return QFEC_OK;
}

bool is_device_ptr(const void* p) {
    if (!p) return false;
    thread_local const void* plain[64] = {};
    const uintptr_t u = (uintptr_t)p;
    const void*& slot = plain[((u >> 4) ^ (u >> 10) ^ (u >> 16)) & 63u];
    if (slot == p) return false;
    hipPointerAttribute_t attr;
    hipError_t e = hipPointerGetAttributes(&attr, p);
    if (e != hipSuccess) {
        (void)hipGetLastError();
        slot = p;
        return false;
    }
    if (attr.type == hipMemoryTypeUnregistered) slot = p;
    return attr.type == hipMemoryTypeDevice || attr.type == hipMemoryTypeManaged;
}

bool is_pinned_host(const void* p) {
    if (!p) return false;
    hipPointerAttribute_t attr;
    hipError_t e = hipPointerGetAttributes(&attr, p);
    if (e != hipSuccess) {
        (void)hipGetLastError();
        return false;
    }
    return attr.type == hipMemoryTypeHost;
}

bool host_dev(const void* h, uint8_t** d) {
    void* p = nullptr;
    if (!h || hipHostGetDevicePointer(&p, const_cast<void*>(h), 0) != hipSuccess || !p) {
        (void)hipGetLastError();
        return false;
    }
    *d = static_cast<uint8_t*>(p);
    return true;
}

int ensure_host_slot(DevCtx::HostSlot& h, size_t in_bytes, size_t out_bytes) {
    if (!h.stream) {
        HIP_TRY(hipStreamCreateWithFlags(&h.stream, hipStreamNonBlocking));
        HIP_TRY(hipEventCreateWithFlags(&h.done, hipEventDisableTiming));
    }
    if (in_bytes > h.in_cap || out_bytes > h.out_cap) {
        if (h.d_buf) HIP_TRY(hipFree(h.d_buf));
        if (h.h_in) HIP_TRY(hipHostFree(h.h_in));
        if (h.h_out) HIP_TRY(hipHostFree(h.h_out));
        h.d_buf = h.h_in = h.h_out = nullptr;
        h.in_cap = h.out_cap = 0;
        HIP_TRY(hipMalloc(&h.d_buf, in_bytes + out_bytes));
        HIP_TRY(hipHostMalloc(&h.h_in, in_bytes, hipHostMallocDefault));
        HIP_TRY(hipHostMalloc(&h.h_out, out_bytes, hipHostMallocDefault));
        h.in_cap = in_bytes;
        h.out_cap = out_bytes;
    }
    return QFEC_OK;
}

void quiesce_host_slots(DevCtx& c) {
    for (auto& h : c.host)
        if (h.stream) (void)hipStreamSynchronize(h.stream);
    (void)hipGetLastError();
}

int gather_rows(DevCtx& c, unsigned char* const* ptrs, size_t count, int len, size_t pitch, uint8_t* d_dst,
                uint8_t* h_tmp, bool dev_src) {
    if (dev_src) {
        for (size_t i = 0; i < count; ++i)
            HIP_TRY(hipMemcpyAsync(d_dst + i * pitch, ptrs[i], (size_t)len, hipMemcpyDefault, c.stream));
        return QFEC_OK;
    }
    for (size_t i = 0; i < count; ++i) memcpy(h_tmp + i * pitch, ptrs[i], (size_t)len);
    HIP_TRY(hipMemcpyAsync(d_dst, h_tmp, count * pitch, hipMemcpyHostToDevice, c.stream));
    return QFEC_OK;
}

int scatter_rows(DevCtx& c, unsigned char* const* ptrs, size_t count, int len, size_t pitch, const uint8_t* d_src,
                 uint8_t* h_tmp, bool dev_dst, const uint8_t* only ) {
    if (dev_dst) {
        for (size_t i = 0; i < count; ++i)
            if (!only || only[i])
                HIP_TRY(hipMemcpyAsync(ptrs[i], d_src + i * pitch, (size_t)len, hipMemcpyDefault, c.stream));
        HIP_TRY(hipStreamSynchronize(c.stream));
        return QFEC_OK;
    }
    HIP_TRY(hipMemcpyAsync(h_tmp, d_src, count * pitch, hipMemcpyDeviceToHost, c.stream));
    HIP_TRY(hipStreamSynchronize(c.stream));
    for (size_t i = 0; i < count; ++i)
        if (!only || only[i]) memcpy(ptrs[i], h_tmp + i * pitch, (size_t)len);
    return QFEC_OK;
}

}


namespace qfec {

qfec_code* make_code(int k, int m, std::vector<uint8_t>&& rows, int quirk) {
    qfec_code* c = new (std::nothrow) qfec_code();
    if (!c) return nullptr;
    c->k = k;
    c->m = m;
    c->quirk = quirk;
    c->rows = std::move(rows);
    return c;
}

void free_code(qfec_code* c) {
    if (!c) return;
    int prev = 0;
    bool have = hipGetDevice(&prev) == hipSuccess;
    for (auto& kv : c->dev) {
        if (hipSetDevice(kv.first) != hipSuccess) continue;
        if (kv.second.d_enc) (void)hipFree(kv.second.d_enc);
        if (kv.second.d_lut) (void)hipFree(kv.second.d_lut);
        if (kv.second.d_rec) (void)hipFree(kv.second.d_rec);
        if (kv.second.d_rep_lut) (void)hipFree(kv.second.d_rep_lut);
        if (kv.second.d_rep_rec) (void)hipFree(kv.second.d_rep_rec);
        if (kv.second.d_loc) (void)hipFree(kv.second.d_loc);
        if (kv.second.d_le_lut) (void)hipFree(kv.second.d_le_lut);
        if (kv.second.d_le_rec) (void)hipFree(kv.second.d_le_rec);
    }
    if (have) (void)hipSetDevice(prev);
    delete c;
}

const uint8_t* full_of(const qfec_code* c) { return c->full.empty() ? nullptr : c->full.data(); }

void enc_table_host(const qfec_code* c, std::vector<uint32_t>& t) {
    const int k = c->k, m = c->m;
    t.assign((size_t)m * k * QFEC_TAB_STRIDE, 0);
    for (int r = 0; r < m; ++r) {
        for (int i = 0; i < k; ++i) perm_entry(c->rows[(size_t)r * k + i], &t[((size_t)r * k + i) * QFEC_TAB_STRIDE]);
        if (c->quirk && c->rows[(size_t)r * k] == 0) t[((size_t)r * k) * QFEC_TAB_STRIDE + 5] = 1;
    }
}

int ensure_enc(qfec_code* c, int dev, uint32_t** out) {
    DevTables& d = c->dev[dev];
    if (d.enc_version != c->version || !d.d_enc) {
        std::vector<uint32_t> t;
        enc_table_host(c, t);
        if (d.d_enc) HIP_TRY(hipFree(d.d_enc));
        d.d_enc = nullptr;
        HIP_TRY(hipMalloc(&d.d_enc, std::max<size_t>(t.size(), 8) * 4));
        if (!t.empty()) HIP_TRY(hipMemcpy(d.d_enc, t.data(), t.size() * 4, hipMemcpyHostToDevice));
        d.enc_version = c->version;
    }
    *out = d.d_enc;
    return QFEC_OK;
}

bool pattern_key(uint64_t mask, int k, int m, uint64_t* key, int* e_out) {
    const uint64_t dm = k >= 64 ? mask : (mask & ((1ull << k) - 1));
    const int e = __builtin_popcountll(dm);
    *e_out = e;
    if (e == 0) { *key = 0; return true; }
    uint64_t avail = ~(mask >> k) & (m >= 64 ? ~0ull : ((1ull << m) - 1));
    uint64_t chosen = 0;
    for (int i = 0; i < e; ++i) {
        if (!avail) return false;
        const uint64_t low = avail & (~avail + 1);
        chosen |= low;
        avail ^= low;
    }
    *key = dm | (chosen << k);
    return true;
}

int record_for_key(const qfec_code* c, uint64_t key, std::vector<uint32_t>& rec) {
    const int k = c->k, m = c->m, n = k + m;
    std::vector<uint8_t> marks(n, 0);
    for (int i = 0; i < k; ++i) marks[i] = (key >> i) & 1;
    for (int j = 0; j < m; ++j) marks[k + j] = ((key >> (k + j)) & 1) ? 0 : 1;
    std::vector<uint8_t> rows;
    std::vector<int> surv, lost;
    const int e = decode_rows(c->rows.data(), k, m, marks.data(), rows, surv, lost, full_of(c));
    if (e <= 0) return -1;
    const RecordLayout L = record_layout(k, m);
    rec.assign(L.words(e, k), 0);
    build_record(L, k, e, rows.data(), surv.data(), lost.data(), c->quirk != 0, rec.data());
    return e;
}

int ensure_lut(qfec_code* c, int dev, DevTables** out) {
    DevTables& d = c->dev[dev];
    *out = &d;
    if (d.rec_version == c->version && d.d_lut) return QFEC_OK;
    const int k = c->k, m = c->m, n = k + m;
    if (n > QFEC_LUT_MAX_N) {
        set_error("qfec_reconstruct: k + m = %d > %d (use reed_solomon_reconstruct)", n, QFEC_LUT_MAX_N);
        return QFEC_EUNSUP;
    }
    const size_t nmask = (size_t)1 << n;
    std::vector<int32_t> lut(nmask);
    std::vector<uint8_t> seed(nmask, 0);
    std::unordered_map<uint64_t, int32_t> off_of;
    std::vector<uint32_t> recs, one;
    for (size_t mask = 0; mask < nmask; ++mask) {
        uint64_t key;
        int e;
        if (!pattern_key(mask, k, m, &key, &e)) { lut[mask] = QFEC_REC_FAIL; continue; }
        if (e == 0) { lut[mask] = QFEC_REC_NONE; continue; }
        auto it = off_of.find(key);
        if (it != off_of.end()) {
            lut[mask] = it->second;
            seed[mask] = recs[(size_t)it->second + 1] != 0;
            continue;
        }
        if (record_for_key(c, key, one) <= 0) { lut[mask] = QFEC_REC_FAIL; continue; }
        one.resize(record_layout(k, m).words(m, k), 0);
        seed[mask] = one[1] != 0;
        const int32_t off = (int32_t)recs.size();
        recs.insert(recs.end(), one.begin(), one.end());
        off_of.emplace(key, off);
        lut[mask] = off;
    }
    if (d.d_lut) HIP_TRY(hipFree(d.d_lut));
    if (d.d_rec) HIP_TRY(hipFree(d.d_rec));
    d.d_lut = nullptr;
    d.d_rec = nullptr;
    HIP_TRY(hipMalloc(&d.d_lut, nmask * 4));
    HIP_TRY(hipMalloc(&d.d_rec, std::max<size_t>(recs.size(), 8) * 4));
    HIP_TRY(hipMemcpy(d.d_lut, lut.data(), nmask * 4, hipMemcpyHostToDevice));
    if (!recs.empty()) HIP_TRY(hipMemcpy(d.d_rec, recs.data(), recs.size() * 4, hipMemcpyHostToDevice));
    d.rec_version = c->version;
    c->lut_seed = std::make_shared<const std::vector<uint8_t>>(std::move(seed));
    c->lut_seed_version = c->version;
    return QFEC_OK;
}

bool vec16_ok(const void* a, const void* b, int block, long long pitch) {
    return ((uintptr_t)a % 16 == 0) && ((uintptr_t)b % 16 == 0) && (pitch % 16 == 0) &&
           (long long)round_up((size_t)block, 16) <= pitch;
}

int run_encode(DevCtx& ctx, const qfec_code* c, const uint32_t* tab, int m, const uint8_t* d_data,
               uint8_t* d_par, long long groups, int block, long long pitch, hipStream_t s, long long dgs,
               long long pgs, bool host_mem) {
    EncodeArgs a{};
    a.tab = tab;
    a.gf_exp = ctx.d_gf;
    a.gf_log = ctx.d_gf + 512;
    a.k = c->k;
    a.m = m;
    a.pitch = (uint64_t)pitch;
    a.vec16 = vec16_ok(d_data, d_par, block, pitch) ? 1 : 0;
    a.impl = tuning().encode_impl;
    a.lds = host_mem ? 0 : tuning().encode_lds.load();
    a.block = host_mem ? 256 : tuning().encode_block.load();
    a.cols = a.vec16 ? (uint32_t)((block + 15) / 16) : (uint32_t)block;
    a.cols_div = make_div_magic(a.cols);
    a.dgs = dgs >= 0 ? (uint64_t)dgs : (uint64_t)c->k * pitch;
    a.pgs = pgs >= 0 ? (uint64_t)pgs : (uint64_t)m * pitch;
    if (a.vec16 && ((a.dgs | a.pgs) & 15)) {
        a.vec16 = 0;
        a.cols = (uint32_t)block;
        a.cols_div = make_div_magic(a.cols);
    }
    const long long per = std::max<long long>(1, (long long)(0x7FFFFFFFll / a.cols));
    for (long long g0 = 0; g0 < groups; g0 += per) {
        const long long gn = std::min(per, groups - g0);
        a.data = d_data + (size_t)g0 * a.dgs;
        a.parity = d_par + (size_t)g0 * a.pgs;
        a.work = (uint64_t)gn * a.cols;
        hipError_t e = launch_encode(a, g_variant.load(), s);
        if (e != hipSuccess) return hip_fail(e, "encode kernel launch");
    }
    return QFEC_OK;
}

int run_reconstruct(DevCtx& ctx, const qfec_code* c, const int32_t* lut, const int32_t* group_rec,
                    const uint32_t* recs, uint8_t* d_data, const uint8_t* d_par, const uint8_t* d_marks,
                    long long groups, int block, long long pitch, unsigned* d_failed, hipStream_t s,
                    long long dgs, long long pgs) {
    ReconArgs a{};
    const RecordLayout L = record_layout(c->k, c->m);
    a.data = d_data;
    a.parity = d_par;
    a.marks = d_marks;
    a.lut = lut;
    a.group_rec = group_rec;
    a.records = recs;
    a.failed = d_failed;
    a.groups = (uint64_t)groups;
    a.pitch = (uint64_t)pitch;
    a.k = c->k;
    a.m = c->m;
    a.surv_off = L.surv_off;
    a.lost_off = L.lost_off;
    a.hdr = L.hdr;
    a.coff = L.coff;
    a.t256 = ctx.d_t256;
    a.dgs = dgs >= 0 ? (uint64_t)dgs : (uint64_t)c->k * pitch;
    a.pgs = pgs >= 0 ? (uint64_t)pgs : (uint64_t)c->m * pitch;
    a.vec16 = vec16_ok(d_data, d_par, block, pitch) && !((a.dgs | a.pgs) & 15) ? 1 : 0;
    a.cols = a.vec16 ? (uint32_t)((block + 15) / 16) : (uint32_t)block;
    a.impl = tuning().recon_impl;
    a.wpg = (a.cols + 63) / 64;
    a.cols8 = (uint32_t)((block + 7) / 8);
    a.cols12 = (uint32_t)((block + 11) / 12);
    if (a.vec16 && c->k < 14) {
        a.cols8 = 2u * a.cols;
        a.cols12 = std::max(a.cols12, a.cols * 16u / 12u);
    }
    a.wpg8 = (a.cols8 + 63) / 64;
    a.wpg12 = (a.cols12 + 63) / 64;
    hipError_t e = launch_reconstruct(a, s);
    if (e != hipSuccess) return hip_fail(e, "reconstruct kernel launch");
    return QFEC_OK;
}

int host_records(qfec_code* c, const uint8_t* marks, long long groups, std::vector<int32_t>& grec,
                 std::vector<uint32_t>& recs, long long* nfail) {
    const int k = c->k, m = c->m;
    if (c->rec_cache_version != c->version) {
        c->rec_cache.clear();
        c->rec_cache_version = c->version;
    }
    std::unordered_map<uint64_t, int32_t> off_of;
    grec.assign((size_t)groups, QFEC_REC_NONE);
    recs.clear();
    *nfail = 0;
    std::vector<uint8_t> gm(k + m);
    for (long long g = 0; g < groups; ++g) {
        const uint8_t* dm = marks + (size_t)g * k;
        const uint8_t* pm = marks + (size_t)groups * k + (size_t)g * m;
        int e = 0;
        for (int i = 0; i < k; ++i) e += dm[i] ? 1 : 0;
        if (!e) continue;
        uint64_t kd = 0;
        std::vector<int> chosen;
        for (int j = 0; j < m && (int)chosen.size() < e; ++j)
            if (!pm[j]) chosen.push_back(j);
        if ((int)chosen.size() < e) { grec[g] = QFEC_REC_FAIL; ++*nfail; continue; }
        uint64_t h = 1469598103934665603ull;
        for (int i = 0; i < k; ++i) if (dm[i]) { h = (h ^ (uint64_t)i) * 1099511628211ull; }
        h = (h ^ 0xFFFFu) * 1099511628211ull;
        for (int j : chosen) h = (h ^ (uint64_t)j) * 1099511628211ull;
        kd = h;
        auto it = off_of.find(kd);
        if (it != off_of.end()) { grec[g] = it->second; continue; }
        auto ct = c->rec_cache.find(kd);
        if (ct == c->rec_cache.end()) {
            for (int i = 0; i < k; ++i) gm[i] = dm[i];
            for (int j = 0; j < m; ++j) gm[k + j] = 1;
            for (int j : chosen) gm[k + j] = 0;
            std::vector<uint8_t> rows;
            std::vector<int> surv, lost;
            const int ee = decode_rows(c->rows.data(), k, m, gm.data(), rows, surv, lost, full_of(c));
            if (ee <= 0) { grec[g] = QFEC_REC_FAIL; ++*nfail; continue; }
            const RecordLayout L = record_layout(k, m);
            std::vector<uint32_t> one(L.words(ee, k));
            build_record(L, k, ee, rows.data(), surv.data(), lost.data(), c->quirk != 0, one.data());
            ct = c->rec_cache.emplace(kd, std::move(one)).first;
        }
        const int32_t off = (int32_t)recs.size();
        recs.insert(recs.end(), ct->second.begin(), ct->second.end());
        off_of.emplace(kd, off);
        grec[g] = off;
    }
    return QFEC_OK;
}

int reconstruct_host_records(DevCtx& ctx, qfec_code* c, uint8_t* d_data, const uint8_t* d_par,
                             const uint8_t* d_marks, long long groups, int block_size, long long pitch,
                             unsigned* d_failed, hipStream_t s) {
    const int n = c->k + c->m;
    std::vector<uint8_t> hm((size_t)groups * n);
    HIP_TRY(hipMemcpyAsync(hm.data(), d_marks, hm.size(), hipMemcpyDeviceToHost, s));
    HIP_TRY(hipStreamSynchronize(s));
    std::vector<int32_t> grec;
    std::vector<uint32_t> recs;
    long long nfail = 0;
    {
        std::lock_guard<std::mutex> lk(c->mu);
        int rc = host_records(c, hm.data(), groups, grec, recs, &nfail);
        if (rc) return rc;
    }
    if (recs.empty() && (!nfail || !d_failed)) return QFEC_OK;
    recs.resize(std::max<size_t>(recs.size(), 8), 0);
    std::lock_guard<std::mutex> lk(ctx.mu);
    const size_t gw = round_up((size_t)groups, 4);
    int rc = ensure_small(ctx, gw + recs.size());
    if (rc) return rc;
    memcpy(ctx.h_small, grec.data(), (size_t)groups * 4);
    memcpy(ctx.h_small + gw, recs.data(), recs.size() * 4);
    HIP_TRY(hipMemcpyAsync(ctx.d_small, ctx.h_small, (gw + recs.size()) * 4, hipMemcpyHostToDevice, s));
    rc = run_reconstruct(ctx, c, nullptr, (const int32_t*)ctx.d_small, ctx.d_small + gw, d_data, d_par, nullptr,
                         groups, block_size, pitch, d_failed, s);
    if (rc) return rc;
    HIP_TRY(hipStreamSynchronize(s));
    return QFEC_OK;
}

}


extern "C" {

const char* qfec_version(void) { return QFEC_VERSION_STRING; }

const char* qfec_last_error(void) { return t_last_error.c_str(); }

const char* qfec_strerror(int err) {
    switch (err) {
        case QFEC_OK: return "ok";
        case QFEC_EINVAL: return "invalid argument";
        case QFEC_ENODEV: return "no HIP device";
        case QFEC_EHIP: return "HIP runtime error";
        case QFEC_ENOMEM: return "out of memory";
        case QFEC_EUNSUP: return "unsupported shape for this entry point";
        default: return "unknown error";
    }
}

int qfec_device_count(void) {
    int n = 0;
    if (hipGetDeviceCount(&n) != hipSuccess) return 0;
    return n;
}

int qfec_set_kernel_variant(int v) {
    if (v != QFEC_VARIANT_PERM && v != QFEC_VARIANT_LDSLOG) return QFEC_EINVAL;
    g_variant.store(v);
    return QFEC_OK;
}

int qfec_get_kernel_variant(void) { return g_variant.load(); }

}

namespace {
struct Knob {
    const char* key;
    std::atomic<int>* v;
    int lo, hi;
};
const std::vector<Knob>& knob_table() {
    static const std::vector<Knob> t = {
        {"recon_impl", &tuning().recon_impl, -1, 8},
        {"host_chunk", &tuning().host_chunk, 0, 0x7FFFFFFF},
        {"host_threads", &tuning().host_threads, 0, 64},
        {"encode_impl", &tuning().encode_impl, -1, 2},
        {"wire_fused", &tuning().wire_fused, 0, 1},
        {"wire_rx", &tuning().wire_rx, 0, 5},
        {"host_zero_copy", &tuning().host_zero_copy, 0, 1},
        {"host_lanes", &tuning().host_lanes, 2, 8},
        {"host_nt", &tuning().host_nt, 0, 2},
        {"percall_fast", &g_percall_fast, 0, 1},
        {"percall_group", &g_percall_group, 0, 1},
        {"percall_fault", &g_percall_fault, 0, 2},
        {"percall_timeout_us", &g_percall_timeout_us, 0, 0x7FFFFFFF},
        {"percall_stop_us", &g_percall_stop_us, 0, 0x7FFFFFFF},
        {"percall_idle_us", &g_percall_idle_us, 0, 1000000},
        {"percall_resident", &g_percall_resident, 0, 1},
        {"encode_lds", &tuning().encode_lds, -1, 163840},
        {"encode_block", &tuning().encode_block, -1, 256},
    };
    return t;
}

void retry_abandoned_servers() {
    for (DevCtx& c : g_ctx) {
        std::lock_guard<std::mutex> lk(c.mu);
        if (c.srv.usable == -2) c.srv.usable = 0;
    }
}

void stop_percall_servers() {
    for (DevCtx& c : g_ctx) {
        std::lock_guard<std::mutex> lk(c.mu);
        if (c.srv.usable <= 0 || !c.srv.launched) continue;
        int prev = 0;
        (void)hipGetDevice(&prev);
        (void)hipSetDevice(c.device);
        (void)pc_server_stop(c);
        (void)hipSetDevice(prev);
    }
}
}

extern "C" {

int qfec_tune(const char* key, int value) {
    if (!key) return QFEC_EINVAL;
    for (const Knob& kn : knob_table()) {
        if (strcmp(key, kn.key)) continue;
        if (value < kn.lo || value > kn.hi) break;
        if (!strcmp(key, "recon_impl") && value != -1 && value != 2 && value != 3 && value != 4 && value != 8) break;
        if (!strcmp(key, "encode_block") && value != -1 && value != 64 && value != 256) break;
        if (!strcmp(key, "encode_impl") && value == 1) break;
        kn.v->store(value);
        if (!strcmp(key, "percall_idle_us") || (!strcmp(key, "percall_resident") && !value)) stop_percall_servers();
        if (!strcmp(key, "percall_resident") && value) retry_abandoned_servers();
        return QFEC_OK;
    }
    set_error("qfec_tune: unknown key/value %s=%d", key, value);
    return QFEC_EINVAL;
}

int qfec_tune_get(const char* key, int* value) {
    if (!key || !value) return QFEC_EINVAL;
    for (const Knob& kn : knob_table())
        if (!strcmp(key, kn.key)) {
            *value = kn.v->load();
            return QFEC_OK;
        }
    set_error("qfec_tune_get: unknown key %s", key);
    return QFEC_EINVAL;
}

int qfec_percall_stats(unsigned long long out[5]) {
    if (!out) return QFEC_EINVAL;
    DevCtx* ctx = nullptr;
    int rc = current_ctx(&ctx);
    if (rc) return rc;
    std::lock_guard<std::mutex> lk(ctx->mu);
    const DevCtx::PcServer& s = ctx->srv;
    out[0] = s.calls;
    out[1] = s.launches;
    out[2] = s.relaunches;
    out[3] = s.usable > 0 && pc_server_alive(s);
    out[4] = (unsigned long long)(long long)s.usable;
    return QFEC_OK;
}


int qfec_percall_counters(unsigned long long* out, int n) {
    if (!out || n < 0) return QFEC_EINVAL;
    unsigned long long v[10] = {0, 0, 0, 0, 0, 0, 0, 0, 0, 0};
    DevCtx* ctx = nullptr;
    int rc = current_ctx(&ctx);
    if (rc) return rc;
    {
        std::lock_guard<std::mutex> lk(ctx->mu);
        const DevCtx::PcServer& s = ctx->srv;
        v[0] = s.calls;
        v[1] = s.launches;
        v[2] = s.relaunches;
        v[3] = s.usable > 0 && pc_server_alive(s);
        v[4] = (unsigned long long)(long long)s.usable;
        v[5] = s.timeouts;
        v[9] = s.abandoned;
    }
    v[6] = g_group_hits.load();
    v[7] = g_group_misses.load();
    v[8] = (unsigned long long)g_percall_idle_us.load();
    for (int i = 0; i < n && i < 10; ++i) out[i] = v[i];
    return std::min(n, 10);
}

qfec_code* qfec_code_new(int flavour, int k, int m) {
    std::vector<uint8_t> rows;
    bool ok = false;
    if (flavour == QFEC_CAUCHY) ok = cauchy_rows(k, m, rows);
    else if (flavour == QFEC_VANDERMONDE) ok = vandermonde_rows(k, m, rows);
    if (!ok) {
        set_error("qfec_code_new: invalid flavour/shape (%d, k=%d, m=%d)", flavour, k, m);
        return nullptr;
    }
    return make_code(k, m, std::move(rows), flavour == QFEC_CAUCHY ? 1 : 0);
}

qfec_code* qfec_code_from_rows(int k, int m, const unsigned char* parity_rows, int rs_stale_quirk) {
    if (k <= 0 || m < 0 || k > 256 || k + m > 256 || (m > 0 && !parity_rows)) {
        set_error("qfec_code_from_rows: bad shape k=%d m=%d", k, m);
        return nullptr;
    }
    std::vector<uint8_t> rows(parity_rows, parity_rows + (size_t)m * k);
    return make_code(k, m, std::move(rows), rs_stale_quirk ? 1 : 0);
}

void qfec_code_free(qfec_code* code) { free_code(code); }

int qfec_code_rows(const qfec_code* code, unsigned char* out) {
    if (!code || !out) return QFEC_EINVAL;
    memcpy(out, code->rows.data(), code->rows.size());
    return QFEC_OK;
}

int qfec_code_shape(const qfec_code* code, int* k, int* m) {
    if (!code) return QFEC_EINVAL;
    if (k) *k = code->k;
    if (m) *m = code->m;
    return QFEC_OK;
}

int qfec_encode(qfec_code* code, const unsigned char* d_data, unsigned char* d_parity, long long groups,
                int block_size, long long pitch, void* stream) {
    if (!code || groups < 0 || block_size < 1 || pitch < block_size || (groups > 0 && (!d_data || !d_parity))) {
        set_error("qfec_encode: invalid argument");
        return QFEC_EINVAL;
    }
    if (groups == 0 || code->m == 0) return QFEC_OK;
    DevCtx* ctx = nullptr;
    int rc = current_ctx(&ctx);
    if (rc) return rc;
    uint32_t* tab = nullptr;
    {
        std::lock_guard<std::mutex> lk(code->mu);
        rc = ensure_enc(code, ctx->device, &tab);
    }
    if (rc) return rc;
    return run_encode(*ctx, code, tab, code->m, d_data, d_parity, groups, block_size, pitch, (hipStream_t)stream);
}

int qfec_encode_host(qfec_code* code, const unsigned char* h_data, unsigned char* h_parity, long long groups,
                     int block_size, long long pitch) {
    if (!code || groups < 0 || block_size < 1 || pitch < block_size || (groups > 0 && (!h_data || !h_parity))) {
        set_error("qfec_encode_host: invalid argument");
        return QFEC_EINVAL;
    }
    if (groups == 0 || code->m == 0) return QFEC_OK;
    DevCtx* ctx = nullptr;
    int rc = current_ctx(&ctx);
    if (rc) return rc;
    uint32_t* tab = nullptr;
    {
        std::lock_guard<std::mutex> lk(code->mu);
        rc = ensure_enc(code, ctx->device, &tab);
    }
    if (rc) return rc;
    const int k = code->k, m = code->m;
    const size_t in_g = (size_t)k * (size_t)pitch, out_g = (size_t)m * (size_t)pitch;
    long long gc = tuning().host_chunk > 0 ? (long long)tuning().host_chunk
                                           : std::max<long long>(1, (long long)((size_t)32 << 20) / (long long)in_g);
    gc = std::min(gc, groups);
    const bool pin_in = is_pinned_host(h_data), pin_out = is_pinned_host(h_parity);
    std::lock_guard<std::mutex> lk(ctx->host_mu);
    uint8_t *z_in = nullptr, *z_out = nullptr;
    if (tuning().host_zero_copy && pin_in && pin_out && host_dev(h_data, &z_in) && host_dev(h_parity, &z_out)) {
        if ((rc = ensure_host_slot(ctx->host[0], 0, 0))) return rc;
        hipStream_t st = ctx->host[0].stream;
        rc = run_encode(*ctx, code, tab, m, z_in, z_out, groups, block_size, pitch, st, -1, -1, true);
        const hipError_t e = hipStreamSynchronize(st);
        if (!rc && e != hipSuccess) rc = hip_fail(e, "qfec_encode_host: zero-copy encode");
        return rc;
    }
    for (int sl = 0; sl < 2; ++sl)
        if ((rc = ensure_host_slot(ctx->host[sl], (size_t)gc * in_g, (size_t)gc * out_g))) return rc;
    long long pending[2] = {-1, -1};
    auto drain = [&](int sl) -> int {
        if (pending[sl] < 0) return QFEC_OK;
        HIP_TRY(hipEventSynchronize(ctx->host[sl].done));
        if (!pin_out) {
            const long long g0 = pending[sl] * gc, gn = std::min(gc, groups - g0);
            memcpy(h_parity + (size_t)g0 * out_g, ctx->host[sl].h_out, (size_t)gn * out_g);
        }
        pending[sl] = -1;
        return QFEC_OK;
    };
    const long long nchunks = (groups + gc - 1) / gc;
    auto chunk = [&](long long i) -> int {
        const int sl = (int)(i & 1);
        DevCtx::HostSlot& h = ctx->host[sl];
        int r = drain(sl);
        if (r) return r;
        const long long g0 = i * gc, gn = std::min(gc, groups - g0);
        const unsigned char* src = h_data + (size_t)g0 * in_g;
        if (!pin_in) {
            memcpy(h.h_in, src, (size_t)gn * in_g);
            src = h.h_in;
        }
        uint8_t* d_in = h.d_buf;
        uint8_t* d_out = h.d_buf + (size_t)gc * in_g;
        HIP_TRY(hipMemcpyAsync(d_in, src, (size_t)gn * in_g, hipMemcpyHostToDevice, h.stream));
        if ((r = run_encode(*ctx, code, tab, m, d_in, d_out, gn, block_size, pitch, h.stream))) return r;
        unsigned char* dst = pin_out ? h_parity + (size_t)g0 * out_g : h.h_out;
        HIP_TRY(hipMemcpyAsync(dst, d_out, (size_t)gn * out_g, hipMemcpyDeviceToHost, h.stream));
        HIP_TRY(hipEventRecord(h.done, h.stream));
        pending[sl] = i;
        return QFEC_OK;
    };
    for (long long i = 0; i < nchunks && !rc; ++i) rc = chunk(i);
    if (!rc) rc = drain((int)(nchunks & 1));
    if (!rc) rc = drain((int)((nchunks + 1) & 1));
    if (rc) quiesce_host_slots(*ctx);
    return rc;
}

int qfec_reconstruct_host(qfec_code* code, unsigned char* h_data, const unsigned char* h_parity,
                          const unsigned char* h_marks, long long groups, int block_size, long long pitch,
                          long long* failed) {
    if (!code || groups < 0 || block_size < 1 || pitch < block_size ||
        (groups > 0 && (!h_data || !h_marks || (code->m > 0 && !h_parity)))) {
        set_error("qfec_reconstruct_host: invalid argument");
        return QFEC_EINVAL;
    }
    if (failed) *failed = 0;
    if (groups == 0) return QFEC_OK;
    const int k = code->k, m = code->m;
    if (k + m > QFEC_LUT_MAX_N) {
        set_error("qfec_reconstruct_host: k + m = %d > %d (use reed_solomon_reconstruct)", k + m, QFEC_LUT_MAX_N);
        return QFEC_EUNSUP;
    }
    DevCtx* ctx = nullptr;
    int rc = current_ctx(&ctx);
    if (rc) return rc;
    DevTables* d = nullptr;
    {
        std::lock_guard<std::mutex> lk(code->mu);
        rc = ensure_lut(code, ctx->device, &d);
    }
    if (rc) return rc;
    const size_t dg = (size_t)k * (size_t)pitch, pg = (size_t)m * (size_t)pitch;
    long long gc = tuning().host_chunk > 0 ? (long long)tuning().host_chunk
                                           : std::max<long long>(1, (long long)((size_t)32 << 20) / (long long)dg);
    gc = std::min(gc, groups);
    const size_t mk_off = (size_t)gc * (dg + pg), cnt_off = round_up(mk_off + (size_t)gc * (k + m), 16);
    const size_t slot_bytes = cnt_off + 16;
    std::lock_guard<std::mutex> lk(ctx->host_mu);
    uint8_t *z_data = nullptr, *z_par = nullptr;
    if (tuning().host_zero_copy && is_pinned_host(h_data) && host_dev(h_data, &z_data) &&
        (m == 0 || (is_pinned_host(h_parity) && host_dev(h_parity, &z_par)))) {
        DevCtx::HostSlot& h = ctx->host[0];
        const size_t mbytes = (size_t)groups * (k + m), zc_cnt = round_up(mbytes, 16);
        if ((rc = ensure_host_slot(h, zc_cnt + 16, zc_cnt + 16))) return rc;
        memcpy(h.h_in, h_marks, mbytes);
        memset(h.h_in + zc_cnt, 0, 16);
        HIP_TRY(hipMemcpyAsync(h.d_buf, h.h_in, zc_cnt + 16, hipMemcpyHostToDevice, h.stream));
        rc = run_reconstruct(*ctx, code, d->d_lut, nullptr, d->d_rec, z_data, z_par, h.d_buf, groups, block_size, pitch,
                             reinterpret_cast<unsigned*>(h.d_buf + zc_cnt), h.stream);
        if (!rc) {
            const hipError_t e1 = hipMemcpyAsync(h.h_out, h.d_buf + zc_cnt, 16, hipMemcpyDeviceToHost, h.stream);
            if (e1 != hipSuccess) rc = hip_fail(e1, "qfec_reconstruct_host: counter");
        }
        const hipError_t e = hipStreamSynchronize(h.stream);
        if (!rc && e != hipSuccess) rc = hip_fail(e, "qfec_reconstruct_host: zero-copy reconstruct");
        if (!rc && failed) *failed = *reinterpret_cast<const unsigned*>(h.h_out);
        return rc;
    }
    for (int sl = 0; sl < 2; ++sl)
        if ((rc = ensure_host_slot(ctx->host[sl], slot_bytes, slot_bytes))) return rc;
    long long pending[2] = {-1, -1};
    long long nfail = 0;
    auto drain = [&](int sl) -> int {
        if (pending[sl] < 0) return QFEC_OK;
        DevCtx::HostSlot& h = ctx->host[sl];
        HIP_TRY(hipEventSynchronize(h.done));
        const long long g0 = pending[sl] * gc, gn = std::min(gc, groups - g0);
        memcpy(h_data + (size_t)g0 * dg, h.h_out, (size_t)gn * dg);
        nfail += *reinterpret_cast<const unsigned*>(h.h_out + cnt_off);
        pending[sl] = -1;
        return QFEC_OK;
    };
    const long long nchunks = (groups + gc - 1) / gc;
    auto chunk = [&](long long i) -> int {
        const int sl = (int)(i & 1);
        DevCtx::HostSlot& h = ctx->host[sl];
        int r = drain(sl);
        if (r) return r;
        const long long g0 = i * gc, gn = std::min(gc, groups - g0);
        memcpy(h.h_in, h_data + (size_t)g0 * dg, (size_t)gn * dg);
        if (m) memcpy(h.h_in + (size_t)gn * dg, h_parity + (size_t)g0 * pg, (size_t)gn * pg);
        uint8_t* hm = h.h_in + (size_t)gn * (dg + pg);
        memcpy(hm, h_marks + (size_t)g0 * k, (size_t)gn * k);
        memcpy(hm + (size_t)gn * k, h_marks + (size_t)groups * k + (size_t)g0 * m, (size_t)gn * m);
        memset(h.h_in + cnt_off, 0, 16);
        const size_t used = (size_t)gn * (dg + pg + k + m);
        uint8_t* dd = h.d_buf;
        HIP_TRY(hipMemcpyAsync(dd, h.h_in, used, hipMemcpyHostToDevice, h.stream));
        HIP_TRY(hipMemcpyAsync(dd + cnt_off, h.h_in + cnt_off, 16, hipMemcpyHostToDevice, h.stream));
        if ((r = run_reconstruct(*ctx, code, d->d_lut, nullptr, d->d_rec, dd, dd + (size_t)gn * dg,
                                 dd + (size_t)gn * (dg + pg), gn, block_size, pitch,
                                 reinterpret_cast<unsigned*>(dd + cnt_off), h.stream)))
            return r;
        HIP_TRY(hipMemcpyAsync(h.h_out, dd, (size_t)gn * dg, hipMemcpyDeviceToHost, h.stream));
        HIP_TRY(hipMemcpyAsync(h.h_out + cnt_off, dd + cnt_off, 16, hipMemcpyDeviceToHost, h.stream));
        HIP_TRY(hipEventRecord(h.done, h.stream));
        pending[sl] = i;
        return QFEC_OK;
    };
    for (long long i = 0; i < nchunks && !rc; ++i) rc = chunk(i);
    if (!rc) rc = drain((int)(nchunks & 1));
    if (!rc) rc = drain((int)((nchunks + 1) & 1));
    if (rc) {
        quiesce_host_slots(*ctx);
        return rc;
    }
    if (failed) *failed = nfail;
    return QFEC_OK;
}

int qfec_prepare_reconstruct(qfec_code* code) {
    if (!code) return QFEC_EINVAL;
    DevCtx* ctx = nullptr;
    int rc = current_ctx(&ctx);
    if (rc) return rc;
    DevTables* d = nullptr;
    std::lock_guard<std::mutex> lk(code->mu);
    return ensure_lut(code, ctx->device, &d);
}

int qfec_reconstruct(qfec_code* code, unsigned char* d_data, const unsigned char* d_parity,
                     const unsigned char* d_marks, long long groups, int block_size, long long pitch,
                     unsigned int* d_failed, void* stream) {
    if (!code || groups < 0 || block_size < 1 || pitch < block_size ||
        (groups > 0 && (!d_data || !d_marks || (code->m > 0 && !d_parity)))) {
        set_error("qfec_reconstruct: invalid argument");
        return QFEC_EINVAL;
    }
    if (groups == 0) return QFEC_OK;
    if (groups > 0x7FFFFFFFll * 4) {
        set_error("qfec_reconstruct: too many groups per call");
        return QFEC_EINVAL;
    }
    DevCtx* ctx = nullptr;
    int rc = current_ctx(&ctx);
    if (rc) return rc;
    if (code->k + code->m > QFEC_LUT_MAX_N) return reconstruct_host_records(*ctx, code, d_data, d_parity, d_marks,
                                                                           groups, block_size, pitch, d_failed,
                                                                           (hipStream_t)stream);
    DevTables* d = nullptr;
    {
        std::lock_guard<std::mutex> lk(code->mu);
        rc = ensure_lut(code, ctx->device, &d);
    }
    if (rc) return rc;
    return run_reconstruct(*ctx, code, d->d_lut, nullptr, d->d_rec, d_data, d_parity, d_marks, groups, block_size,
                           pitch, d_failed, (hipStream_t)stream);
}

int qfec_decode_rows(const qfec_code* code, const unsigned char* marks_n, unsigned char* rows_out,
                     int* survivors_out, int* erased_out) {
    if (!code || !marks_n) return QFEC_EINVAL;
    std::vector<uint8_t> rows;
    std::vector<int> surv, lost;
    const int e = decode_rows(code->rows.data(), code->k, code->m, marks_n, rows, surv, lost, full_of(code));
    if (e > 0) {
        if (rows_out) memcpy(rows_out, rows.data(), rows.size());
        if (survivors_out) memcpy(survivors_out, surv.data(), surv.size() * sizeof(int));
        if (erased_out) memcpy(erased_out, lost.data(), lost.size() * sizeof(int));
    }
    return e;
}

int qfec_synth_fill(unsigned char* d_ptr, long long nbytes, unsigned long long seed, void* stream) {
    if (nbytes < 0 || (nbytes > 0 && !d_ptr)) return QFEC_EINVAL;
    DevCtx* ctx = nullptr;
    int rc = current_ctx(&ctx);
    if (rc) return rc;
    hipError_t e = launch_synth_fill(d_ptr, (uint64_t)nbytes, seed, (hipStream_t)stream);
    return e == hipSuccess ? QFEC_OK : hip_fail(e, "synth fill launch");
}

int qfec_probe_stream(const unsigned char* d_data, unsigned char* d_parity, long long groups, int k, int m,
                      int block_size, long long pitch, void* stream) {
    if (groups <= 0 || k <= 0 || m <= 0 || !vec16_ok(d_data, d_parity, block_size, pitch)) return QFEC_EINVAL;
    DevCtx* ctx = nullptr;
    int rc = current_ctx(&ctx);
    if (rc) return rc;
    EncodeArgs a{};
    a.data = d_data;
    a.parity = d_parity;
    a.k = k;
    a.m = m;
    a.pitch = (uint64_t)pitch;
    a.vec16 = 1;
    a.cols = (uint32_t)((block_size + 15) / 16);
    a.cols_div = make_div_magic(a.cols);
    a.work = (uint64_t)groups * a.cols;
    a.dgs = (uint64_t)k * pitch;
    a.pgs = (uint64_t)m * pitch;
    a.lds = tuning().encode_lds.load();
    a.block = tuning().encode_block.load();
    if (a.work >= 0x80000000ull) return QFEC_EINVAL;
    hipError_t e = launch_probe_xor(a, (hipStream_t)stream);
    return e == hipSuccess ? QFEC_OK : hip_fail(e, "probe launch");
}

int qfec_probe_reconstruct(unsigned char* d_data, const unsigned char* d_parity, const unsigned char* d_marks,
                           long long groups, int k, int m, int block_size, long long pitch, int lds_cap,
                           void* stream) {
    if (groups <= 0 || !d_marks || lds_cap < 0 || lds_cap > 163840 || !vec16_ok(d_data, d_parity, block_size, pitch))
        return QFEC_EINVAL;
    if (!((k == 10 && m == 3) || (k == 16 && m == 4))) return QFEC_EUNSUP;
    DevCtx* ctx = nullptr;
    int rc = current_ctx(&ctx);
    if (rc) return rc;
    ReconArgs a{};
    a.data = d_data;
    a.parity = d_parity;
    a.marks = d_marks;
    a.groups = (uint64_t)groups;
    a.pitch = (uint64_t)pitch;
    a.k = k;
    a.m = m;
    a.dgs = (uint64_t)k * pitch;
    a.pgs = (uint64_t)m * pitch;
    a.cols = (uint32_t)((block_size + 15) / 16);
    a.cols8 = k < 14 ? 2u * a.cols : (uint32_t)((block_size + 7) / 8);
    a.wpg8 = (a.cols8 + 63) / 64;
    a.rlds = lds_cap;
    hipError_t e = launch_probe_recon(a, (hipStream_t)stream);
    return e == hipSuccess ? QFEC_OK : hip_fail(e, "reconstruct probe launch");
}

}
```

Measured before the change: 4549.

## Specialize encode/reconstruct kernels to drop quirk reloads and use 32-bit row offsets

Adds a compile-time QUIRK template flag to the encode, reconstruct and repair kernels. When the host finds that no table entry needs the legacy 'quirk' seed reload, the kernels skip the conditional read of existing destination contents. Row addressing moves to 32-bit offsets through a GroupRows helper, with a fallback to the generic kernel when rows do not fit in 32 bits. The per-wave group division is replaced by a magic-number divide, and there are new recon_order and recon_lds tuning knobs. This cuts extra global loads and 64-bit address arithmetic at the cost of more template instantiations and extra host-side bookkeeping.

```diff
diff --git a/quicknet_amd/csrc/gf256.cpp b/quicknet_amd/csrc/gf256.cpp
--- a/quicknet_amd/csrc/gf256.cpp
+++ b/quicknet_amd/csrc/gf256.cpp
@@ -46,6 +46,8 @@
     static Tuning t;
     return t;
 }
+
+int recon_order_resolved() { return tuning().recon_order.load() == 1 ? 1 : 0; }
 
 const Field& field() {
     std::call_once(g_field_once, build_field);
diff --git a/quicknet_amd/csrc/qfec_internal.hpp b/quicknet_amd/csrc/qfec_internal.hpp
--- a/quicknet_amd/csrc/qfec_internal.hpp
+++ b/quicknet_amd/csrc/qfec_internal.hpp
@@ -43,6 +43,7 @@
     int impl;
     int lds;
     int block;
+    int quirk;
 };
 
 struct ReconArgs {
@@ -67,6 +68,9 @@
     uint32_t cols8, wpg8;
     uint32_t cols12, wpg12;
     int rlds;
+    int quirk;
+    int order;
+    DivMagic wdiv;
 };
 
 struct RepairArgs {
@@ -86,6 +90,9 @@
     int k, m;
     int surv_off, lost_off, coff;
     int vec16;
+    int quirk;
+    int order;
+    DivMagic wdiv;
 };
 
 struct VerifyArgs {
@@ -241,7 +248,10 @@
     std::atomic<int> host_nt{2};
     std::atomic<int> encode_block{-1};
     std::atomic<int> encode_lds{-1};
-};
+    std::atomic<int> recon_lds{0};
+    std::atomic<int> recon_order{-1};
+};
+int recon_order_resolved();
 Tuning& tuning();
 
 hipError_t launch_encode(const EncodeArgs& a, int variant, hipStream_t stream);
diff --git a/quicknet_amd/csrc/qfec_kernels.hip b/quicknet_amd/csrc/qfec_kernels.hip
--- a/quicknet_amd/csrc/qfec_kernels.hip
+++ b/quicknet_amd/csrc/qfec_kernels.hip
@@ -12,7 +12,7 @@
 namespace qfec {
 
 
-template <int K, int M, int BS = 256>
+template <int K, int M, int BS = 256, bool QUIRK = true>
 __global__ void __launch_bounds__(256) k_encode_perm(EncodeArgs a) {
     const uint64_t t = (uint64_t)blockIdx.x * (uint64_t)BS + threadIdx.x;
     if (t >= a.work) return;
@@ -30,7 +30,8 @@
 #pragma unroll
     for (int r = 0; r < M; ++r) {
         acc[r] = make_uint4(0, 0, 0, 0);
-        if (tab[(r * K) * QFEC_TAB_STRIDE + 5]) acc[r] = *reinterpret_cast<const uint4*>(dst + (uint64_t)r * a.pitch);
+        if constexpr (QUIRK)
+            if (tab[(r * K) * QFEC_TAB_STRIDE + 5]) acc[r] = *reinterpret_cast<const uint4*>(dst + (uint64_t)r * a.pitch);
     }
 #pragma unroll
     for (int c = 0; c + 1 < K; c += 2) {
@@ -51,7 +52,7 @@
     for (int r = 0; r < M; ++r) st16(dst + (uint64_t)r * a.pitch, acc[r]);
 }
 
-template <int K, int M, int BS = 256>
+template <int K, int M, int BS = 256, bool QUIRK = true>
 __global__ void __launch_bounds__(256) k_encode_perm_halves(EncodeArgs a) {
     constexpr int H = (K + 1) / 2;
     const uint64_t t = (uint64_t)blockIdx.x * (uint64_t)BS + threadIdx.x;
@@ -65,7 +66,8 @@
 #pragma unroll
     for (int r = 0; r < M; ++r) {
         acc[r] = make_uint4(0, 0, 0, 0);
-        if (tab[(r * K) * QFEC_TAB_STRIDE + 5]) acc[r] = *reinterpret_cast<const uint4*>(dst + (uint64_t)r * a.pitch);
+        if constexpr (QUIRK)
+            if (tab[(r * K) * QFEC_TAB_STRIDE + 5]) acc[r] = *reinterpret_cast<const uint4*>(dst + (uint64_t)r * a.pitch);
     }
 #pragma unroll
     for (int c0 = 0; c0 < K; c0 += H) {
@@ -236,15 +238,42 @@
         __builtin_nontemporal_store(t, reinterpret_cast<u32x2*>(p));
     }
 }
+template <int ROWS>
+__device__ __forceinline__ void body_starts_here(uint32_t& off) {
+    asm volatile("; %1-row body" : "+v"(off) : "n"(ROWS) : "memory");
+}
 template <int D>
 __device__ __forceinline__ void ldv_plain(uint32_t (&v)[D], const uint8_t* p) {
 #pragma unroll
     for (int d = 0; d < D; ++d) v[d] = reinterpret_cast<const uint32_t*>(p)[d];
 }
 
-template <int K, int E, int D>
-__device__ __forceinline__ void recon_column_e(const uint8_t* const (&src)[K], uint8_t* __restrict__ data_g,
-                                               uint64_t lost_bits, const RTab& T, uint64_t pitch, uint64_t off) {
+struct GroupRows {
+    uint8_t* data_g;
+    uint8_t* par_g;
+    uint32_t pitch;
+    __device__ __forceinline__ GroupRows(uint8_t* data, const uint8_t* parity, uint64_t g, uint64_t dgs, uint64_t pgs,
+                                         uint32_t pitch_)
+        : data_g(data + g * dgs), par_g(const_cast<uint8_t*>(parity) + g * pgs), pitch(pitch_) {}
+    __device__ __forceinline__ uint8_t* row(uint32_t s, uint32_t K) const {
+        return (s < K ? data_g : par_g) + (uint32_t)((s < K ? s : s - K) * pitch);
+    }
+};
+
+template <int K>
+__device__ __forceinline__ void survivor_rows(const uint8_t* (&src)[K], const GroupRows& R, uint64_t avail) {
+#pragma unroll
+    for (int c = 0; c < K; ++c) {
+        const uint32_t s = (uint32_t)__builtin_ctzll(avail);
+        avail &= avail - 1;
+        src[c] = R.row(s, K);
+    }
+}
+
+template <int K, int E, int D, bool QUIRK>
+__device__ __forceinline__ void recon_column_e(const uint8_t* const (&src)[K], const GroupRows& R, uint64_t lost_bits,
+                                               const RTab& T, uint32_t off) {
+    if constexpr (!QUIRK) body_starts_here<E>(off);
     uint32_t x[K][D];
 #pragma unroll
     for (int c = 0; c < K; ++c) ldv<D>(x[c], src[c] + off);
@@ -254,38 +283,54 @@
     for (int j = 0; j < E; ++j) {
         const uint32_t l = (uint32_t)__builtin_ctzll(lost_bits);
         lost_bits &= lost_bits - 1;
-        dst[j] = data_g + (uint64_t)l * pitch + off;
+        dst[j] = R.row(l, K) + off;
 #pragma unroll
         for (int d = 0; d < D; ++d) acc[j][d] = 0;
-        if (T.quirk(j, K)) ldv_plain<D>(acc[j], dst[j]);
+        if constexpr (QUIRK)
+            if (T.quirk(j, K)) ldv_plain<D>(acc[j], dst[j]);
     }
     recon_mac_core<K, E, D>(x, acc, T);
 #pragma unroll
     for (int j = 0; j < E; ++j) stv<D>(dst[j], acc[j]);
 }
 
-template <int K, int M, int D, int E = M>
-__device__ __forceinline__ void recon_column_by_e(const uint8_t* const (&src)[K], uint8_t* __restrict__ data_g,
-                                                  uint64_t lost_bits, const RTab& T, int e, uint64_t pitch, uint64_t off) {
+template <int K, int M, int D, bool QUIRK, int E = M>
+__device__ __forceinline__ void recon_column_by_e(const uint8_t* const (&src)[K], const GroupRows& R,
+                                                  uint64_t lost_bits, const RTab& T, int e, uint32_t off) {
     if constexpr (E > 1) {
         if (e < E) {
-            recon_column_by_e<K, M, D, E - 1>(src, data_g, lost_bits, T, e, pitch, off);
+            recon_column_by_e<K, M, D, QUIRK, E - 1>(src, R, lost_bits, T, e, off);
             return;
         }
     }
-    recon_column_e<K, E, D>(src, data_g, lost_bits, T, pitch, off);
-}
-
-template <int K, int M, int IMPL>
+    recon_column_e<K, E, D, QUIRK>(src, R, lost_bits, T, off);
+}
+
+__device__ __forceinline__ uint32_t fast_div32(uint32_t n, const DivMagic& d) {
+    if (d.pow2) return n >> d.shift;
+    const uint64_t hi = (uint64_t)n * (uint32_t)(d.mul >> 32) + __umulhi(n, (uint32_t)d.mul);
+    return (uint32_t)(hi >> d.shift);
+}
+
+template <int K, int M, int IMPL, bool ONE, bool QUIRK>
 __device__ __forceinline__ void recon_item(const ReconArgs& a, uint8_t* __restrict__ data,
                                            const uint8_t* __restrict__ parity, const uint8_t* __restrict__ marks,
                                            const int32_t* __restrict__ lut, const uint32_t* __restrict__ records,
-                                           uint32_t wid, int lane) {
+                                           int lane) {
     constexpr int N = K + M;
-    const uint32_t wpg = IMPL == 3 ? a.wpg8 : IMPL == 4 ? a.wpg12 : a.wpg;
-    const uint64_t g = wid / wpg;
-    const uint32_t part = wid - (uint32_t)g * wpg;
-    if (g >= a.groups) return;
+    const uint32_t wave = __builtin_amdgcn_readfirstlane(threadIdx.x >> 6);
+    uint32_t gi, part;
+    if constexpr (ONE) {
+        gi = blockIdx.x;
+        part = wave;
+    } else {
+        const uint32_t wpg = IMPL == 3 ? a.wpg8 : IMPL == 4 ? a.wpg12 : a.wpg;
+        const uint32_t wid = blockIdx.x * 4u + wave;
+        gi = fast_div32(wid, a.wdiv);
+        part = wid - gi * wpg;
+    }
+    if (gi >= a.groups) return;
+    const uint64_t g = a.order ? a.groups - 1u - gi : (uint64_t)gi;
     uint32_t mk = 0;
     if (lane < K) mk = marks[g * K + lane];
     else if (lane < N) mk = marks[a.groups * K + g * M + (lane - K)];
@@ -293,41 +338,32 @@
     const uint64_t lost_bits = mask & ((1ull << K) - 1ull);
     const int e = __builtin_popcountll(lost_bits);
     if (e == 0) return;
-    uint64_t avail = ~mask & ((1ull << N) - 1ull);
+    const uint64_t avail = ~mask & ((1ull << N) - 1ull);
     if (__builtin_popcountll(avail) < K) {
         if (part == 0 && lane == 0 && a.failed) atomicAdd(a.failed, 1u);
         return;
     }
     const int rec = ((const __attribute__((address_space(4))) int32_t*)lut)[mask];
     const RTab T{records + rec, a.coff, a.t256};
-    const uint64_t pitch = a.pitch;
-    uint8_t* data_g = data + g * a.dgs;
-    const uint8_t* par_g = parity + g * a.pgs;
+    const GroupRows R(data, parity, g, a.dgs, a.pgs, (uint32_t)a.pitch);
     const uint8_t* src[K];
-#pragma unroll
-    for (int c = 0; c < K; ++c) {
-        const uint32_t s = (uint32_t)__builtin_ctzll(avail);
-        avail &= avail - 1;
-        src[c] = s < (uint32_t)K ? data_g + (uint64_t)s * pitch : par_g + (uint64_t)(s - K) * pitch;
-    }
+    survivor_rows<K>(src, R, avail);
     const uint32_t col = part * 64u + lane;
     if (col < (IMPL == 3 ? a.cols8 : IMPL == 4 ? a.cols12 : a.cols)) {
-        if (IMPL == 2) recon_column_by_e<K, M, 4>(src, data_g, lost_bits, T, e, pitch, (uint64_t)col * 16u);
-        else if (IMPL == 3) recon_column_by_e<K, M, 2>(src, data_g, lost_bits, T, e, pitch, (uint64_t)col * 8u);
-        else recon_column_by_e<K, M, 3>(src, data_g, lost_bits, T, e, pitch, (uint64_t)col * 12u);
-    }
-}
-
-template <int K, int M, int IMPL_>
+        if (IMPL == 2) recon_column_by_e<K, M, 4, QUIRK>(src, R, lost_bits, T, e, col * 16u);
+        else if (IMPL == 3) recon_column_by_e<K, M, 2, QUIRK>(src, R, lost_bits, T, e, col * 8u);
+        else recon_column_by_e<K, M, 3, QUIRK>(src, R, lost_bits, T, e, col * 12u);
+    }
+}
+
+template <int K, int M, int IMPL_, bool QUIRK = true>
 __global__ void __launch_bounds__(256) k_reconstruct_perm(ReconArgs a, uint8_t* __restrict__ data,
                                                           const uint8_t* __restrict__ parity,
                                                           const uint8_t* __restrict__ marks,
                                                           const int32_t* __restrict__ lut,
                                                           const uint32_t* __restrict__ records) {
     constexpr int IMPL = IMPL_ == 8 ? 3 : IMPL_;
-    const int lane = threadIdx.x & 63;
-    const uint32_t wid = __builtin_amdgcn_readfirstlane(blockIdx.x * (IMPL_ == 8 ? a.wpg8 : 4u) + (threadIdx.x >> 6));
-    recon_item<K, M, IMPL>(a, data, parity, marks, lut, records, wid, lane);
+    recon_item<K, M, IMPL, IMPL_ == 8, QUIRK>(a, data, parity, marks, lut, records, threadIdx.x & 63);
 }
 
 template <bool VEC16>
@@ -398,10 +434,10 @@
 }
 
 
-template <int K, int T, int D>
-__device__ __forceinline__ void repair_column_t(const uint8_t* const (&src)[K], uint8_t* __restrict__ data_g,
-                                                uint8_t* __restrict__ par_g, uint64_t lost_bits, const RTab& R,
-                                                uint64_t pitch, uint64_t off) {
+template <int K, int T, int D, bool QUIRK>
+__device__ __forceinline__ void repair_column_t(const uint8_t* const (&src)[K], const GroupRows& G, uint64_t lost_bits,
+                                                const RTab& R, uint32_t off) {
+    if constexpr (!QUIRK) body_starts_here<T>(off);
     uint32_t x[K][D];
 #pragma unroll
     for (int c = 0; c < K; ++c) ldv<D>(x[c], src[c] + off);
@@ -411,30 +447,30 @@
     for (int j = 0; j < T; ++j) {
         const uint32_t l = (uint32_t)__builtin_ctzll(lost_bits);
         lost_bits &= lost_bits - 1;
-        dst[j] = (l < (uint32_t)K ? data_g + (uint64_t)l * pitch : par_g + (uint64_t)(l - K) * pitch) + off;
+        dst[j] = G.row(l, K) + off;
 #pragma unroll
         for (int d = 0; d < D; ++d) acc[j][d] = 0;
-        if (R.quirk(j, K)) ldv_plain<D>(acc[j], dst[j]);
+        if constexpr (QUIRK)
+            if (R.quirk(j, K)) ldv_plain<D>(acc[j], dst[j]);
     }
     recon_mac_core<K, T, D>(x, acc, R);
 #pragma unroll
     for (int j = 0; j < T; ++j) stv<D>(dst[j], acc[j]);
 }
 
-template <int K, int M, int D, int T = M>
-__device__ __forceinline__ void repair_column_by_t(const uint8_t* const (&src)[K], uint8_t* __restrict__ data_g,
-                                                   uint8_t* __restrict__ par_g, uint64_t lost_bits, const RTab& R,
-                                                   int t, uint64_t pitch, uint64_t off) {
+template <int K, int M, int D, bool QUIRK, int T = M>
+__device__ __forceinline__ void repair_column_by_t(const uint8_t* const (&src)[K], const GroupRows& G,
+                                                   uint64_t lost_bits, const RTab& R, int t, uint32_t off) {
     if constexpr (T > 1) {
         if (t < T) {
-            repair_column_by_t<K, M, D, T - 1>(src, data_g, par_g, lost_bits, R, t, pitch, off);
+            repair_column_by_t<K, M, D, QUIRK, T - 1>(src, G, lost_bits, R, t, off);
             return;
         }
     }
-    repair_column_t<K, T, D>(src, data_g, par_g, lost_bits, R, pitch, off);
-}
-
-template <int K, int M, bool ONE>
+    repair_column_t<K, T, D, QUIRK>(src, G, lost_bits, R, off);
+}
+
+template <int K, int M, bool ONE, bool QUIRK = true>
 __global__ void __launch_bounds__(256) k_repair_perm(RepairArgs a, uint8_t* __restrict__ data,
                                                      uint8_t* __restrict__ parity,
                                                      const uint8_t* __restrict__ dmarks,
@@ -444,17 +480,17 @@
     constexpr int N = K + M;
     const int lane = threadIdx.x & 63;
     const uint32_t wave = __builtin_amdgcn_readfirstlane(threadIdx.x >> 6);
-    uint64_t g;
-    uint32_t part;
+    uint32_t gi, part;
     if (ONE) {
-        g = blockIdx.x;
+        gi = blockIdx.x;
         part = wave;
     } else {
         const uint32_t wid = blockIdx.x * 4u + wave;
-        g = wid / a.wpg8;
-        part = wid - (uint32_t)g * a.wpg8;
-    }
-    if (g >= a.groups) return;
+        gi = fast_div32(wid, a.wdiv);
+        part = wid - gi * a.wpg8;
+    }
+    if (gi >= a.groups) return;
+    const uint64_t g = a.order ? a.groups - 1u - gi : (uint64_t)gi;
     uint32_t mk = 0;
     if (lane < K) mk = dmarks[g * K + lane];
     else if (lane < N) mk = pmarks[g * M + (lane - K)];
@@ -471,19 +507,11 @@
         return;
     }
     const RTab R{records + rec, a.coff, a.t256};
-    const uint64_t pitch = a.pitch;
-    uint8_t* data_g = data + g * a.dgs;
-    uint8_t* par_g = parity + g * a.pgs;
-    uint64_t avail = ~mask & ((1ull << N) - 1ull);
+    const GroupRows G(data, parity, g, a.dgs, a.pgs, (uint32_t)a.pitch);
     const uint8_t* src[K];
-#pragma unroll
-    for (int c = 0; c < K; ++c) {
-        const uint32_t s = (uint32_t)__builtin_ctzll(avail);
-        avail &= avail - 1;
-        src[c] = s < (uint32_t)K ? data_g + (uint64_t)s * pitch : par_g + (uint64_t)(s - K) * pitch;
-    }
+    survivor_rows<K>(src, G, ~mask & ((1ull << N) - 1ull));
     const uint32_t col = part * 64u + lane;
-    if (col < a.cols8) repair_column_by_t<K, M, 2>(src, data_g, par_g, mask, R, t, pitch, (uint64_t)col * 8u);
+    if (col < a.cols8) repair_column_by_t<K, M, 2, QUIRK>(src, G, mask, R, t, col * 8u);
 }
 
 template <bool VEC16>
@@ -607,7 +635,7 @@
 __global__ void __launch_bounds__(256) k_probe_recon(ReconArgs a) {
     constexpr int N = K + M;
     const int lane = threadIdx.x & 63;
-    const uint64_t g = blockIdx.x;
+    const uint64_t g = a.order ? a.groups - 1u - blockIdx.x : (uint64_t)blockIdx.x;
     const uint32_t part = __builtin_amdgcn_readfirstlane(threadIdx.x >> 6);
     uint32_t mk = 0;
     if (lane < K) mk = a.marks[g * K + lane];
@@ -660,6 +688,8 @@
     return (unsigned)((work + block - 1) / block);
 }
 
+static inline bool rows_fit_32(int n, uint64_t pitch) { return (uint64_t)n * pitch <= 0xFFFFFFFFull; }
+
 static inline unsigned enc_block(const EncodeArgs& a, int K, int im) {
     if (a.block == 64 || a.block == 256) return (unsigned)a.block;
     const bool lines = (a.pitch % 128 == 0) && (a.dgs % 128 == 0) && (a.pgs % 128 == 0) &&
@@ -676,19 +706,25 @@
     return 40960;
 }
 
+template <int K, int M, bool QUIRK>
+static void enc_launch(const EncodeArgs& a, int im, unsigned bs, unsigned grid, size_t lds, hipStream_t stream) {
+    if (im == 2 && bs == 64)
+        hipLaunchKernelGGL((k_encode_perm_halves<K, M, 64, QUIRK>), dim3(grid_for(a.work, 64)), dim3(64), lds, stream, a);
+    else if (im == 2)
+        hipLaunchKernelGGL((k_encode_perm_halves<K, M, 256, QUIRK>), dim3(grid), dim3(256), lds, stream, a);
+    else if (bs == 64)
+        hipLaunchKernelGGL((k_encode_perm<K, M, 64, QUIRK>), dim3(grid_for(a.work, 64)), dim3(64), lds, stream, a);
+    else
+        hipLaunchKernelGGL((k_encode_perm<K, M, 256, QUIRK>), dim3(grid), dim3(256), lds, stream, a);
+}
+
 #define QFEC_ENC_CASE(KK, MM)                                                                 \
     if (a.k == KK && a.m == MM) {                                                             \
         const int im = a.impl < 0 ? (KK >= 16 ? 2 : 0) : a.impl;                              \
         const unsigned bs = enc_block(a, KK, im);                                             \
         const size_t lds = enc_lds(a, KK, im, grid, bs);                                      \
-        if (im == 2 && bs == 64)                                                              \
-            hipLaunchKernelGGL((k_encode_perm_halves<KK, MM, 64>), dim3(grid_for(a.work, 64)), dim3(64), lds, stream, a); \
-        else if (im == 2)                                                                     \
-            hipLaunchKernelGGL((k_encode_perm_halves<KK, MM>), dim3(grid), dim3(256), lds, stream, a); \
-        else if (bs == 64)                                                                    \
-            hipLaunchKernelGGL((k_encode_perm<KK, MM, 64>), dim3(grid_for(a.work, 64)), dim3(64), lds, stream, a); \
-        else                                                                                  \
-            hipLaunchKernelGGL((k_encode_perm<KK, MM>), dim3(grid), dim3(256), lds, stream, a);  \
+        if (a.quirk) enc_launch<KK, MM, true>(a, im, bs, grid, lds, stream);                  \
+        else enc_launch<KK, MM, false>(a, im, bs, grid, lds, stream);                         \
         return hipGetLastError();                                                             \
     }
 
@@ -723,11 +759,18 @@
     return hipGetLastError();
 }
 
-#define QFEC_REC_LAUNCH(KK, MM, AR)                                                                        \
-    do {                                                                                                   \
-        const dim3 blk(AR == 8 ? 64u * a.wpg8 : 256u), grd(AR == 8 ? (unsigned)a.groups : pgrid);          \
-        hipLaunchKernelGGL((k_reconstruct_perm<KK, MM, AR>), grd, blk, 0, stream, a, a.data, a.parity, a.marks, \
-                           a.lut, a.records);                                                              \
+template <int K, int M, int AR, bool QUIRK>
+static void rec_launch(ReconArgs a, unsigned pgrid, hipStream_t stream) {
+    const dim3 blk(AR == 8 ? 64u * a.wpg8 : 256u), grd(AR == 8 ? (unsigned)a.groups : pgrid);
+    a.wdiv = make_div_magic(AR == 3 ? a.wpg8 : AR == 4 ? a.wpg12 : a.wpg);
+    hipLaunchKernelGGL((k_reconstruct_perm<K, M, AR, QUIRK>), grd, blk, (size_t)std::max(a.rlds, 0), stream, a, a.data,
+                       a.parity, a.marks, a.lut, a.records);
+}
+
+#define QFEC_REC_LAUNCH(KK, MM, AR)                                          \
+    do {                                                                     \
+        if (a.quirk) rec_launch<KK, MM, AR, true>(a, pgrid, stream);         \
+        else rec_launch<KK, MM, AR, false>(a, pgrid, stream);                \
     } while (0)
 
 #define QFEC_REC_CASE(KK, MM)                                                      \
@@ -763,6 +806,10 @@
     }
     const uint64_t waves = a.groups * (uint64_t)std::max(std::max(a.wpg, a.wpg8), a.wpg12);
     if (waves > 0xFFFFFFFFull) return hipErrorInvalidValue;
+    if (!rows_fit_32(a.k + a.m, a.pitch)) {
+        hipLaunchKernelGGL((k_reconstruct_any<true>), dim3(grid), dim3(256), 0, stream, a);
+        return hipGetLastError();
+    }
     const unsigned pgrid16 = grid_for(a.groups * (uint64_t)a.wpg, 4);
     const unsigned pgrid8 = grid_for(a.groups * (uint64_t)a.wpg8, 4);
     const unsigned pgrid12 = grid_for(a.groups * (uint64_t)a.wpg12, 4);
@@ -787,15 +834,22 @@
     return hipGetLastError();
 }
 
-#define QFEC_REP_CASE(KK, MM)                                                                                   \
-    if (a.k == KK && a.m == MM) {                                                                               \
-        if (a.wpg8 >= 1 && a.wpg8 <= 4)                                                                         \
-            hipLaunchKernelGGL((k_repair_perm<KK, MM, true>), dim3((unsigned)a.groups), dim3(64u * a.wpg8), 0, \
-                               stream, a, a.data, a.parity, a.dmarks, a.pmarks, a.lut, a.records);              \
-        else                                                                                                    \
-            hipLaunchKernelGGL((k_repair_perm<KK, MM, false>), dim3(grid_for(a.groups * (uint64_t)a.wpg8, 4)), \
-                               dim3(256), 0, stream, a, a.data, a.parity, a.dmarks, a.pmarks, a.lut, a.records); \
-        return hipGetLastError();                                                                               \
+template <int K, int M, bool QUIRK>
+static void rep_launch(RepairArgs a, hipStream_t stream) {
+    a.wdiv = make_div_magic(a.wpg8);
+    if (a.wpg8 >= 1 && a.wpg8 <= 4)
+        hipLaunchKernelGGL((k_repair_perm<K, M, true, QUIRK>), dim3((unsigned)a.groups), dim3(64u * a.wpg8), 0, stream,
+                           a, a.data, a.parity, a.dmarks, a.pmarks, a.lut, a.records);
+    else
+        hipLaunchKernelGGL((k_repair_perm<K, M, false, QUIRK>), dim3(grid_for(a.groups * (uint64_t)a.wpg8, 4)),
+                           dim3(256), 0, stream, a, a.data, a.parity, a.dmarks, a.pmarks, a.lut, a.records);
+}
+
+#define QFEC_REP_CASE(KK, MM)                                 \
+    if (a.k == KK && a.m == MM) {                             \
+        if (a.quirk) rep_launch<KK, MM, true>(a, stream);     \
+        else rep_launch<KK, MM, false>(a, stream);            \
+        return hipGetLastError();                             \
     }
 
 hipError_t launch_repair(const RepairArgs& a, hipStream_t stream) {
@@ -805,6 +859,10 @@
     const unsigned grid = grid_for(a.groups, 4);
     if (!a.vec16) {
         hipLaunchKernelGGL((k_repair_any<false>), dim3(grid), dim3(256), 0, stream, a);
+        return hipGetLastError();
+    }
+    if (!rows_fit_32(a.k + a.m, a.pitch)) {
+        hipLaunchKernelGGL((k_repair_any<true>), dim3(grid), dim3(256), 0, stream, a);
         return hipGetLastError();
     }
     QFEC_REP_CASE(10, 3)
diff --git a/quicknet_amd/csrc/qfec_repair.cpp b/quicknet_amd/csrc/qfec_repair.cpp
--- a/quicknet_amd/csrc/qfec_repair.cpp
+++ b/quicknet_amd/csrc/qfec_repair.cpp
@@ -13,6 +13,7 @@
     std::vector<uint32_t> recs;
     std::vector<uint8_t> marks((size_t)n), rows;
     std::vector<int> surv, lost;
+    bool any_seed = false;
     for (size_t mask = 0; mask < nmask; ++mask) {
         const int t = __builtin_popcountll((unsigned long long)mask);
         if (t == 0) { lut[mask] = QFEC_REC_NONE; continue; }
@@ -26,6 +27,7 @@
         const size_t off = recs.size();
         recs.resize(off + (size_t)L.hdr);
         build_repair_record(L, k, t, e, rows.data(), surv.data(), lost.data(), c->quirk != 0, &recs[off]);
+        any_seed |= recs[off + 1] != 0;
         lut[mask] = (int32_t)off;
     }
     if (d.d_rep_lut) HIP_TRY(hipFree(d.d_rep_lut));
@@ -37,6 +39,8 @@
     HIP_TRY(hipMemcpy(d.d_rep_lut, lut.data(), nmask * 4, hipMemcpyHostToDevice));
     if (!recs.empty()) HIP_TRY(hipMemcpy(d.d_rep_rec, recs.data(), recs.size() * 4, hipMemcpyHostToDevice));
     d.rep_version = c->version;
+    c->rep_any_seed = any_seed;
+    c->rep_seed_version = c->version;
     return QFEC_OK;
 }
 
@@ -64,6 +68,8 @@
     a.dgs = (uint64_t)c->k * pitch;
     a.pgs = (uint64_t)c->m * pitch;
     a.vec16 = vec16_ok(d_data, d_par, block, pitch) ? 1 : 0;
+    a.quirk = c->quirk && (c->rep_seed_version != c->version || c->rep_any_seed) ? 1 : 0;
+    a.order = recon_order_resolved();
     a.cols = a.vec16 ? (uint32_t)((block + 15) / 16) : (uint32_t)block;
     a.cols8 = a.vec16 && c->k < 14 ? 2u * a.cols : (uint32_t)((block + 7) / 8);
     a.wpg8 = (a.cols8 + 63) / 64;
diff --git a/quicknet_amd/csrc/qfec_rt.hpp b/quicknet_amd/csrc/qfec_rt.hpp
--- a/quicknet_amd/csrc/qfec_rt.hpp
+++ b/quicknet_amd/csrc/qfec_rt.hpp
@@ -147,6 +147,9 @@
     uint64_t rec_cache_version = ~0ull;
     std::shared_ptr<const std::vector<uint8_t>> lut_seed;
     uint64_t lut_seed_version = ~0ull;
+    bool lut_any_seed = true;
+    bool rep_any_seed = true;
+    uint64_t rep_seed_version = ~0ull;
     uint64_t le_host_version = ~0ull;
     int le_rc = 0;
     std::string le_error;
diff --git a/quicknet_amd/csrc/qfec_runtime.cpp b/quicknet_amd/csrc/qfec_runtime.cpp
--- a/quicknet_amd/csrc/qfec_runtime.cpp
+++ b/quicknet_amd/csrc/qfec_runtime.cpp
@@ -280,6 +280,13 @@
     }
 }
 
+static bool enc_any_stale(const qfec_code* c) {
+    if (!c->quirk) return false;
+    for (size_t r = 0; r < (size_t)c->m && (r + 1) * (size_t)c->k <= c->rows.size(); ++r)
+        if (c->rows[r * (size_t)c->k] == 0) return true;
+    return false;
+}
+
 int ensure_enc(qfec_code* c, int dev, uint32_t** out) {
     DevTables& d = c->dev[dev];
     if (d.enc_version != c->version || !d.d_enc) {
@@ -341,6 +348,7 @@
     std::vector<uint8_t> seed(nmask, 0);
     std::unordered_map<uint64_t, int32_t> off_of;
     std::vector<uint32_t> recs, one;
+    bool any_seed = false;
     for (size_t mask = 0; mask < nmask; ++mask) {
         uint64_t key;
         int e;
@@ -355,6 +363,7 @@
         if (record_for_key(c, key, one) <= 0) { lut[mask] = QFEC_REC_FAIL; continue; }
         one.resize(record_layout(k, m).words(m, k), 0);
         seed[mask] = one[1] != 0;
+        any_seed |= one[1] != 0;
         const int32_t off = (int32_t)recs.size();
         recs.insert(recs.end(), one.begin(), one.end());
         off_of.emplace(key, off);
@@ -371,6 +380,7 @@
     d.rec_version = c->version;
     c->lut_seed = std::make_shared<const std::vector<uint8_t>>(std::move(seed));
     c->lut_seed_version = c->version;
+    c->lut_any_seed = any_seed;
     return QFEC_OK;
 }
 
@@ -393,6 +403,7 @@
     a.impl = tuning().encode_impl;
     a.lds = host_mem ? 0 : tuning().encode_lds.load();
     a.block = host_mem ? 256 : tuning().encode_block.load();
+    a.quirk = enc_any_stale(c) ? 1 : 0;
     a.cols = a.vec16 ? (uint32_t)((block + 15) / 16) : (uint32_t)block;
     a.cols_div = make_div_magic(a.cols);
     a.dgs = dgs >= 0 ? (uint64_t)dgs : (uint64_t)c->k * pitch;
@@ -441,6 +452,9 @@
     a.vec16 = vec16_ok(d_data, d_par, block, pitch) && !((a.dgs | a.pgs) & 15) ? 1 : 0;
     a.cols = a.vec16 ? (uint32_t)((block + 15) / 16) : (uint32_t)block;
     a.impl = tuning().recon_impl;
+    a.quirk = c->quirk && (c->lut_seed_version != c->version || c->lut_any_seed) ? 1 : 0;
+    a.order = recon_order_resolved();
+    a.rlds = tuning().recon_lds.load();
     a.wpg = (a.cols + 63) / 64;
     a.cols8 = (uint32_t)((block + 7) / 8);
     a.cols12 = (uint32_t)((block + 11) / 12);
@@ -601,6 +615,8 @@
         {"percall_resident", &g_percall_resident, 0, 1},
         {"encode_lds", &tuning().encode_lds, -1, 163840},
         {"encode_block", &tuning().encode_block, -1, 256},
+        {"recon_order", &tuning().recon_order, -1, 1},
+        {"recon_lds", &tuning().recon_lds, 0, 163840},
     };
     return t;
 }
@@ -1037,6 +1053,7 @@
     a.cols8 = k < 14 ? 2u * a.cols : (uint32_t)((block_size + 7) / 8);
     a.wpg8 = (a.cols8 + 63) / 64;
     a.rlds = lds_cap;
+    a.order = recon_order_resolved();
     hipError_t e = launch_probe_recon(a, (hipStream_t)stream);
     return e == hipSuccess ? QFEC_OK : hip_fail(e, "reconstruct probe launch");
 }
```

After: 4533. Within noise of the previous version (-0.3%).
